# jrnerupudinho/Semi-Blind-Channel-Estimation-for-MIMO-RIS-communication-system-Using-EM-Algo

Hardware: NVIDIA B200
Metric: EM channel-estimation trials/sec (higher is better)
Workload: dtype f64

## Files before the change

semi-blind-channel-estimation-for-mimo-ris-communication-system-using-em-algo_b200/csrc/abi.cu:

```cuda
#include <atomic>
#include <mutex>
#include <vector>
#include <stdio.h>
#include <string.h>

#include "common.cuh"

namespace sbce {

static std::atomic<long long> g_launches{0};
void count_launch(int n) { g_launches.fetch_add(n, std::memory_order_relaxed); }

struct PhaseSpan { int phase; cudaEvent_t a, b; };
static std::atomic<bool> g_prof_on{false};
static std::vector<PhaseSpan> g_spans;
static std::vector<cudaEvent_t> g_event_pool;
static std::mutex g_prof_mu;

static cudaEvent_t prof_event() {
    {
        std::lock_guard<std::mutex> lock(g_prof_mu);
        if (!g_event_pool.empty()) { cudaEvent_t e = g_event_pool.back(); g_event_pool.pop_back(); return e; }
    }
    cudaEvent_t e;
    cudaEventCreate(&e);
    return e;
}

struct PhaseScope {
    bool on; int phase; cudaStream_t s; cudaEvent_t a;
    PhaseScope(int ph, cudaStream_t st) : on(g_prof_on.load(std::memory_order_relaxed)), phase(ph), s(st), a(nullptr) {
        if (on) { a = prof_event(); cudaEventRecord(a, s); }
    }
    ~PhaseScope() {
        if (on) {
            cudaEvent_t b = prof_event();
            cudaEventRecord(b, s);
            std::lock_guard<std::mutex> lock(g_prof_mu);
            g_spans.push_back({phase, a, b});
        }
    }
};

static int make_dims(const sbce_cfg* c, Dims* d, bool with_estep = true) {
    if (!c) return SBCE_E_NULL;
    if (c->N < 1 || c->n_tx < 1 || c->n_rx < 1 || c->T_p < 0 || c->T_d < 1 || c->itera < 0 || c->batch < 0)
        return SBCE_E_SHAPE;
    int sq = 0;
    if (c->M == 4) sq = 2; else if (c->M == 16) sq = 4; else if (c->M == 64) sq = 8; else return SBCE_E_UNSUPPORTED;
    if (c->n_tx > 8 || c->n_rx > 8) return SBCE_E_UNSUPPORTED;
    if (!gram_supports(c->N + 1, c->n_tx, c->n_rx)) return SBCE_E_UNSUPPORTED;
    if (c->n_tx <= 4 && !(c->n_rx <= 4 || c->n_rx == 6 || c->n_rx == 8)) return SBCE_E_UNSUPPORTED;
    if (c->mode < SBCE_MODE_SOFT || c->mode > SBCE_MODE_MMSE) return SBCE_E_UNSUPPORTED;
    if (with_estep) {
        const int bits = c->n_tx * (sq == 2 ? 2 : (sq == 4 ? 4 : 6));
        const bool tree = c->mode == SBCE_MODE_SOFT || c->mode == SBCE_MODE_HARD;
        if (tree && c->n_tx > 4 && bits > 24) return SBCE_E_UNSUPPORTED;
        if ((c->mode == SBCE_MODE_ZF || c->mode == SBCE_MODE_MMSE) && bits > 30) return SBCE_E_UNSUPPORTED;
    }
    d->N = c->N; d->N1 = c->N + 1; d->n_tx = c->n_tx; d->n_rx = c->n_rx; d->M = c->M; d->sqM = sq;
    d->bitsM = (sq == 2 ? 2 : (sq == 4 ? 4 : 6));
    d->T_p = c->T_p; d->T_d = c->T_d; d->itera = c->itera;
    d->L = d->N1 * c->n_tx;
    d->Lp = (d->L + 7) & ~7;
    d->RP = (c->n_rx + 3) & ~3;
    d->Ltot = d->Lp + d->RP;
    d->mode = c->mode; d->flags = c->flags; d->p1 = c->partition_p1;
    d->psi_shared = (c->flags & SBCE_FLAG_PSI_SHARED) ? 1 : 0;
    d->psiP_shared = (c->flags & (SBCE_FLAG_PSI_SHARED | SBCE_FLAG_PSIP_SHARED)) ? 1 : 0;
    d->rec = qr_record_doubles(c->n_tx);
    if (c->mode == SBCE_MODE_PM || c->mode == SBCE_MODE_PM_BETA) {
        if (c->partition_p1 < 1 || c->partition_p1 > c->n_tx) return SBCE_E_SHAPE;
    }
    if (c->mode >= SBCE_MODE_PM && c->n_rx < c->n_tx) return SBCE_E_UNSUPPORTED;
    if (c->flags & SBCE_FLAG_SUPERIMPOSED) {
        if (c->T_p != 0) return SBCE_E_SHAPE;
        if (c->mode != SBCE_MODE_SOFT && c->mode != SBCE_MODE_HARD) return SBCE_E_UNSUPPORTED;
    }
    return 0;
}

static inline size_t al(size_t x) { return (x + 255) & ~(size_t)255; }

size_t carve_workspace(const Dims& d, int nb, void* base, Workspace* ws) {
    size_t off = 0;
    char* p = (char*)base;
    auto take = [&](size_t bytes) { char* r = p ? p + off : nullptr; off += al(bytes); return r; };
    const size_t B = (size_t)nb;
    ws->stat_m = (double*)take(B * d.T_d * d.n_tx * 16);
    ws->stat_R = (double*)take(B * d.T_d * d.n_tx * d.n_tx * 16);
    ws->pil_m = (double*)take(B * d.T_p * d.n_tx * 16 + 16);
    ws->pil_R = (double*)take(B * d.T_p * d.n_tx * d.n_tx * 16 + 16);
    ws->qr = (double*)take(B * d.T_d * d.rec * 8);
    ws->lse_sym = (double*)take(B * d.T_d * 8);
    ws->Gp = (double*)take(B * d.Ltot * d.Lp * 16);
    ws->G = (double*)take(B * d.Ltot * d.Lp * 16);
    ws->active = (int32_t*)take(B * 4);
    ws->stat = (int32_t*)take(B * 4);
    ws->kscratch = (int32_t*)take(B * d.T_d * 4);
    ws->thbuf = (double*)take(B * d.Lp * d.n_rx * 16);
    ws->psiw = (double*)take(B * d.T_p * d.N1 * 16 + 16);
    ws->ls_scale = (double*)take(B * d.N1 * 8);
    ws->ls_rep = (int32_t*)take(B * d.N1 * 4);
    ws->bytes = off;
    return off;
}

#define CK(x)                                  \
    do {                                       \
        cudaError_t _e = (x);                  \
        if (_e != cudaSuccess) return (int)_e; \
    } while (0)

cudaError_t launch_pm_stats(const Dims& d, int nb, const double* Yd, const double* PsiD, const double* theta,
                            const double* varn, const int32_t* active, double* stat_m, double* stat_R,
                            int32_t* kstar, cudaStream_t s);

static int estep_dispatch(const Dims& d, int nb, const double* Yd, const double* PsiD, const double* theta,
                          const double* varn, const int32_t* active, Workspace& ws, double* stat_m, double* stat_R,
                          int32_t* kstar, double* lse_sym, const double* Xoff, cudaStream_t s) {
    if (d.mode == SBCE_MODE_SOFT || d.mode == SBCE_MODE_HARD) {
        {
            PhaseScope ps(SBCE_PHASE_HEFF_QR, s);
            CK(launch_heff_qr(d, nb, Yd, PsiD, theta, active, Xoff, ws.qr, s));
        }
        {
            PhaseScope ps(SBCE_PHASE_ENUM, s);
            CK(launch_enum(d, nb, ws.qr, varn, active, stat_m, stat_R, kstar, lse_sym, s));
            if (Xoff) CK(launch_superimpose_stats(d, nb, Xoff, active, stat_m, stat_R, s));
        }
    } else {
        PhaseScope ps(SBCE_PHASE_ENUM, s);
        CK(launch_pm_stats(d, nb, Yd, PsiD, theta, varn, active, stat_m, stat_R, kstar, s));
    }
    return 0;
}

static inline Dims pilot_dims(const Dims& d) { Dims dp = d; dp.psi_shared = d.psiP_shared; return dp; }

static int em_chunk(const Dims& d, int nb, const sbce_io& io, Workspace& ws, cudaStream_t s) {
    const bool tree = d.mode == SBCE_MODE_SOFT || d.mode == SBCE_MODE_HARD;
    const bool decides = tree || d.mode == SBCE_MODE_ZF || d.mode == SBCE_MODE_MMSE;
    if (io.kstar && !decides) CK(cudaMemsetAsync(io.kstar, 0xFF, (size_t)nb * d.T_d * sizeof(int32_t), s));
    {
        PhaseScope ps(SBCE_PHASE_SETUP, s);
        CK(launch_init_state(d, nb, io.theta0, io.theta, ws.active, ws.stat, io.iters, io.llf, io.lse, s));
        CK(launch_pilot_stats(d, nb, io.Xp, ws.pil_m, ws.pil_R, s));
        CK(launch_normal_equations(pilot_dims(d), nb, io.PsiP, d.T_p, io.Yp, ws.pil_m, ws.pil_R, nullptr, ws.Gp, nullptr, s));
    }
    for (int l = 0; l < d.itera; ++l) {
        int rc = estep_dispatch(d, nb, io.Yd, io.PsiD, io.theta, io.varn, ws.active, ws, ws.stat_m, ws.stat_R,
                                io.kstar, ws.lse_sym, (d.flags & SBCE_FLAG_SUPERIMPOSED) ? io.Xp : nullptr, s);
        if (rc) return rc;
        {
            PhaseScope ps(SBCE_PHASE_GRAM, s);
            CK(launch_normal_equations(d, nb, io.PsiD, d.T_d, io.Yd, ws.stat_m, ws.stat_R, ws.Gp, ws.G, ws.active,
                                       s));
        }
        {
            PhaseScope ps(SBCE_PHASE_CHOL, s);
            CK(launch_chol_solve(d, nb, ws.G, io.theta, ws.active, ws.stat, ws.thbuf, s));
        }
        {
            PhaseScope ps(SBCE_PHASE_METRICS, s);
            CK(launch_after_iteration(d, nb, l, io.theta, io.h_true, io.Yp, io.Yd, io.PsiP, io.PsiD, io.Xp,
                                      io.Xd_true, io.varn, tree ? ws.lse_sym : nullptr, ws.active, io.iters, io.llf,
                                      io.lse, s));
        }
    }
    {
        PhaseScope ps(SBCE_PHASE_METRICS, s);
        CK(launch_final_metrics(d, nb, io.theta, io.h_true, ws.stat, io.nmse, io.status, s));
    }
    return 0;
}

static sbce_io offset_io(const Dims& d, const sbce_io& io, size_t b0) {
    sbce_io o = io;
    const size_t Ln = (size_t)d.L * d.n_rx * 2;
    auto adv = [](const double* p, size_t n) { return p ? p + n : p; };
    auto advw = [](double* p, size_t n) { return p ? p + n : p; };
    o.Yd = adv(io.Yd, b0 * d.T_d * d.n_rx * 2);
    o.Yp = adv(io.Yp, b0 * d.T_p * d.n_rx * 2);
    if (!d.psi_shared) o.PsiD = adv(io.PsiD, b0 * d.T_d * d.N1 * 2);
    if (!d.psiP_shared) o.PsiP = adv(io.PsiP, b0 * d.T_p * d.N1 * 2);
    o.Xp = adv(io.Xp, b0 * ((d.flags & SBCE_FLAG_SUPERIMPOSED) ? d.T_d : d.T_p) * d.n_tx * 2);
    o.theta0 = adv(io.theta0, b0 * Ln);
    o.varn = adv(io.varn, b0);
    o.h_true = adv(io.h_true, b0 * Ln);
    o.Xd_true = adv(io.Xd_true, b0 * d.T_d * d.n_tx * 2);
    o.theta = advw(io.theta, b0 * Ln);
    o.kstar = io.kstar ? io.kstar + b0 * d.T_d : nullptr;
    o.llf = advw(io.llf, b0 * d.itera);
    o.lse = advw(io.lse, b0 * d.itera);
    o.nmse = advw(io.nmse, b0);
    o.iters = io.iters ? io.iters + b0 : nullptr;
    o.status = io.status ? io.status + b0 : nullptr;
    return o;
}

static int check_io(const Dims& d, const sbce_io* io) {
    if (!io) return SBCE_E_NULL;
    if (!io->Yd || !io->PsiD || !io->varn || !io->theta) return SBCE_E_NULL;
    if (d.T_p > 0 && (!io->Yp || !io->PsiP || !io->Xp)) return SBCE_E_NULL;
    if (!(d.flags & SBCE_FLAG_ZERO_START) && !io->theta0) return SBCE_E_NULL;
    if ((d.flags & SBCE_FLAG_GENIE_STOP) && !io->h_true) return SBCE_E_NULL;
    if ((d.flags & SBCE_FLAG_SUPERIMPOSED) && !io->Xp) return SBCE_E_NULL;
    return 0;
}

}

using namespace sbce;

extern "C" {

int sbce_version(void) { return SBCE_VERSION; }

const char* sbce_error_string(int code) {
    switch (code) {
        case 0: return "ok";
        case SBCE_E_NULL: return "required pointer is null";
        case SBCE_E_SHAPE: return "invalid shape parameter";
        case SBCE_E_UNSUPPORTED: return "unsupported configuration (n_tx,n_rx<=8; n_tx<=4: n_rx in {1,2,3,4,6,8}; M in {4,16,64}; N+1+n_tx^2<=908; exhaustive modes with n_tx>4 need n_tx*log2(M)<=24)";
        case SBCE_E_WORKSPACE: return "workspace too small for one trial";
        case SBCE_E_NODEVICE: return "no CUDA device";
        default: return code > 0 ? cudaGetErrorString((cudaError_t)code) : "unknown error";
    }
}

int sbce_device_count(void) {
    int n = 0;
    if (cudaGetDeviceCount(&n) != cudaSuccess) { cudaGetLastError(); return 0; }
    return n;
}

int sbce_workspace_bytes(const sbce_cfg* cfg, int32_t trials_in_flight, size_t* bytes) {
    Dims d;
    int rc = make_dims(cfg, &d);
    if (rc) return rc;
    if (!bytes) return SBCE_E_NULL;
    if (trials_in_flight < 1) return SBCE_E_SHAPE;
    Workspace ws;
    *bytes = carve_workspace(d, trials_in_flight, nullptr, &ws);
    return 0;
}

constexpr int SBCE_MAX_CHUNK = 65535;
static int trials_fitting(const Dims& d, size_t bytes, int want) {
    Workspace ws;
    if (want > SBCE_MAX_CHUNK) want = SBCE_MAX_CHUNK;
    if (carve_workspace(d, 1, nullptr, &ws) > bytes) return 0;
    int lo = 1, hi = want;
    while (lo < hi) {
        int mid = (lo + hi + 1) / 2;
        if (carve_workspace(d, mid, nullptr, &ws) <= bytes) lo = mid; else hi = mid - 1;
    }
    return lo;
}

int sbce_em_batch(const sbce_cfg* cfg, const sbce_io* io, void* workspace, size_t workspace_bytes, void* stream) {
    Dims d;
    int rc = make_dims(cfg, &d);
    if (rc) return rc;
    rc = check_io(d, io);
    if (rc) return rc;
    if (cfg->batch == 0) return 0;
    if (!workspace) return SBCE_E_NULL;
    const int chunk = trials_fitting(d, workspace_bytes, cfg->batch);
    if (chunk < 1) return SBCE_E_WORKSPACE;
    cudaStream_t s = (cudaStream_t)stream;
    for (int b0 = 0; b0 < cfg->batch; b0 += chunk) {
        const int nb = (cfg->batch - b0 < chunk) ? cfg->batch - b0 : chunk;
        Workspace ws;
        carve_workspace(d, nb, workspace, &ws);
        sbce_io o = offset_io(d, *io, (size_t)b0);
        rc = em_chunk(d, nb, o, ws, s);
        if (rc) return rc;
    }
    return 0;
}

int sbce_estep(const sbce_cfg* cfg, const sbce_io* io, const double* theta, double* stat_m, double* stat_R,
               int32_t* kstar, double* lse_sym, void* workspace, size_t workspace_bytes, void* stream) {
    Dims d;
    int rc = make_dims(cfg, &d);
    if (rc) return rc;
    if (!io || !io->Yd || !io->PsiD || !io->varn || !theta || !stat_m || !stat_R || !workspace) return SBCE_E_NULL;
    if (cfg->batch == 0) return 0;
    const int chunk = trials_fitting(d, workspace_bytes, cfg->batch);
    if (chunk < 1) return SBCE_E_WORKSPACE;
    cudaStream_t s = (cudaStream_t)stream;
    for (int b0 = 0; b0 < cfg->batch; b0 += chunk) {
        const int nb = (cfg->batch - b0 < chunk) ? cfg->batch - b0 : chunk;
        Workspace ws;
        carve_workspace(d, nb, workspace, &ws);
        sbce_io o = offset_io(d, *io, (size_t)b0);
        const size_t sb = (size_t)b0 * d.T_d;
        rc = estep_dispatch(d, nb, o.Yd, o.PsiD, theta + (size_t)b0 * d.L * d.n_rx * 2, o.varn, nullptr, ws,
                            stat_m + sb * d.n_tx * 2, stat_R + sb * d.n_tx * d.n_tx * 2, kstar ? kstar + sb : nullptr,
                            lse_sym ? lse_sym + sb : nullptr, (d.flags & SBCE_FLAG_SUPERIMPOSED) ? o.Xp : nullptr, s);
        if (rc) return rc;
    }
    return 0;
}

int sbce_mstep(const sbce_cfg* cfg, const sbce_io* io, const double* stat_m, const double* stat_R, double* theta_out,
               int32_t* status, void* workspace, size_t workspace_bytes, void* stream) {
    Dims d;
    int rc = make_dims(cfg, &d, false);
    if (rc) return rc;
    if (!io || !io->Yd || !io->PsiD || !stat_m || !stat_R || !theta_out || !workspace) return SBCE_E_NULL;
    if (d.T_p > 0 && (!io->Yp || !io->PsiP || !io->Xp)) return SBCE_E_NULL;
    if (cfg->batch == 0) return 0;
    const int chunk = trials_fitting(d, workspace_bytes, cfg->batch);
    if (chunk < 1) return SBCE_E_WORKSPACE;
    cudaStream_t s = (cudaStream_t)stream;
    for (int b0 = 0; b0 < cfg->batch; b0 += chunk) {
        const int nb = (cfg->batch - b0 < chunk) ? cfg->batch - b0 : chunk;
        Workspace ws;
        carve_workspace(d, nb, workspace, &ws);
        sbce_io o = offset_io(d, *io, (size_t)b0);
        const size_t sb = (size_t)b0 * d.T_d;
        CK(cudaMemsetAsync(ws.stat, 0, (size_t)nb * 4, s));
        CK(launch_pilot_stats(d, nb, o.Xp, ws.pil_m, ws.pil_R, s));
        CK(launch_normal_equations(pilot_dims(d), nb, o.PsiP, d.T_p, o.Yp, ws.pil_m, ws.pil_R, nullptr, ws.Gp, nullptr, s));
        CK(launch_normal_equations(d, nb, o.PsiD, d.T_d, o.Yd, stat_m + sb * d.n_tx * 2,
                                   stat_R + sb * d.n_tx * d.n_tx * 2, ws.Gp, ws.G, nullptr, s));
        CK(launch_chol_solve(d, nb, ws.G, theta_out + (size_t)b0 * d.L * d.n_rx * 2, nullptr, ws.stat, ws.thbuf, s));
        if (status) CK(cudaMemcpyAsync(status + b0, ws.stat, (size_t)nb * 4, cudaMemcpyDeviceToDevice, s));
    }
    return 0;
}

int sbce_accumulate_nmse(const double* nmse, const int32_t* status, int32_t batch, double* acc, void* stream) {
    if (!nmse || !acc) return SBCE_E_NULL;
    CK(launch_accumulate_nmse(nmse, status, batch, acc, (cudaStream_t)stream));
    return 0;
}

int sbce_generate_batch(const sbce_cfg* cfg, const sbce_gen* gen, const sbce_io* io, void* stream) {
    Dims d;
    int rc = make_dims(cfg, &d, false);
    if (rc) return rc;
    if (!gen || !io) return SBCE_E_NULL;
    if (!io->h_true || !io->Xd_true || !io->PsiD || !io->Yd || !io->varn) return SBCE_E_NULL;
    if (d.T_p > 0 && (!io->Xp || !io->PsiP || !io->Yp)) return SBCE_E_NULL;
    if (gen->pilot_design < SBCE_PILOTS_PM || gen->pilot_design > SBCE_PILOTS_TOP) return SBCE_E_UNSUPPORTED;
    if (gen->data_phases < SBCE_PHASES_RANDOM || gen->data_phases > SBCE_PHASES_DFT) return SBCE_E_UNSUPPORTED;
    if (cfg->batch == 0) return 0;
    for (int b0 = 0; b0 < cfg->batch; b0 += SBCE_MAX_CHUNK) {
        const int nb = (cfg->batch - b0 < SBCE_MAX_CHUNK) ? cfg->batch - b0 : SBCE_MAX_CHUNK;
        sbce_gen g = *gen;
        g.trial0 = gen->trial0 + b0;
        const sbce_io o = offset_io(d, *io, (size_t)b0);
        CK(launch_generate(d, nb, &g, o, (double*)o.h_true, (double*)o.Xp, (double*)o.Xd_true, (double*)o.PsiP,
                           (double*)o.PsiD, (double*)o.Yp, (double*)o.Yd, (cudaStream_t)stream));
    }
    return 0;
}

int sbce_ls_start(const sbce_cfg* cfg, const sbce_io* io, double* theta0, int32_t* status, void* workspace,
                  size_t workspace_bytes, void* stream) {
    Dims d;
    int rc = make_dims(cfg, &d, false);
    if (rc) return rc;
    if (!io || !io->Yp || !io->PsiP || !io->Xp || !theta0 || !workspace) return SBCE_E_NULL;
    if (d.T_p < 1) return SBCE_E_SHAPE;
    if (cfg->batch == 0) return 0;
    const int chunk = trials_fitting(d, workspace_bytes, cfg->batch);
    if (chunk < 1) return SBCE_E_WORKSPACE;
    for (int b0 = 0; b0 < cfg->batch; b0 += chunk) {
        const int nb = (cfg->batch - b0 < chunk) ? cfg->batch - b0 : chunk;
        Workspace ws;
        carve_workspace(d, nb, workspace, &ws);
        sbce_io o = offset_io(d, *io, (size_t)b0);
        CK(launch_ls_start(pilot_dims(d), nb, o, theta0 + (size_t)b0 * d.L * d.n_rx * 2, status ? status + b0 : nullptr, ws,
                           (cudaStream_t)stream));
    }
    return 0;
}

int sbce_accumulate_ser(const sbce_cfg* cfg, const int32_t* kstar, const double* Xd_true, int32_t batch, double* acc,
                        void* stream) {
    Dims d;
    int rc = make_dims(cfg, &d, false);
    if (rc) return rc;
    if (!kstar || !Xd_true || !acc) return SBCE_E_NULL;
    if (d.n_tx * d.bitsM > 30) return SBCE_E_UNSUPPORTED;
    CK(launch_accumulate_ser(d, batch, kstar, Xd_true, acc, (cudaStream_t)stream));
    return 0;
}

int sbce_measure_fp64_peak(double* tflops, double* seconds) {
    CK(run_fp64_peak(tflops, seconds));
    return 0;
}

int sbce_profile_begin(void) {
    std::lock_guard<std::mutex> lock(g_prof_mu);
    for (auto& sp : g_spans) { g_event_pool.push_back(sp.a); g_event_pool.push_back(sp.b); }
    g_spans.clear();
    g_prof_on.store(true);
    return 0;
}

int sbce_profile_end(double* ms_per_phase, int64_t* spans_per_phase, int32_t n_phases) {
    std::lock_guard<std::mutex> lock(g_prof_mu);
    g_prof_on.store(false);
    if (!ms_per_phase || n_phases < 1) return SBCE_E_NULL;
    for (int i = 0; i < n_phases; ++i) { ms_per_phase[i] = 0.0; if (spans_per_phase) spans_per_phase[i] = 0; }
    for (auto& sp : g_spans) {
        CK(cudaEventSynchronize(sp.b));
        float ms = 0.f;
        CK(cudaEventElapsedTime(&ms, sp.a, sp.b));
        if (sp.phase >= 0 && sp.phase < n_phases) {
            ms_per_phase[sp.phase] += ms;
            if (spans_per_phase) spans_per_phase[sp.phase] += 1;
        }
        g_event_pool.push_back(sp.a);
        g_event_pool.push_back(sp.b);
    }
    g_spans.clear();
    return 0;
}

int64_t sbce_launch_count(int32_t reset) {
    long long v = g_launches.load();
    if (reset) g_launches.store(0);
    return (int64_t)v;
}

namespace {
struct GraphSlot {
    unsigned long long key = 0;
    int seen = 0;
    long long launches = 0;
    cudaGraphExec_t exec = nullptr;
    unsigned long long stamp = 0;
};
struct DevPool {
    void* p = nullptr;
    size_t cap = 0;
    cudaStream_t stream = nullptr;
    cudaStream_t copy = nullptr;
    cudaEvent_t ev[2] = {nullptr, nullptr};
    GraphSlot graphs[4];
    unsigned long long clock = 0;
    std::mutex mu;
};

unsigned long long fnv1a(const void* data, size_t n, unsigned long long h) {
    const unsigned char* p = (const unsigned char*)data;
    for (size_t i = 0; i < n; ++i) { h ^= p[i]; h *= 1099511628211ull; }
    return h;
}
constexpr int SBCE_MAX_DEVICES = 64;
DevPool g_pool[SBCE_MAX_DEVICES];

int pool_get(int dev, size_t bytes, DevPool** out) {
    DevPool& P = g_pool[dev];
    if (!P.stream) {
        CK(cudaStreamCreateWithFlags(&P.stream, cudaStreamNonBlocking));
        CK(cudaStreamCreateWithFlags(&P.copy, cudaStreamNonBlocking));
        CK(cudaEventCreateWithFlags(&P.ev[0], cudaEventDisableTiming));
        CK(cudaEventCreateWithFlags(&P.ev[1], cudaEventDisableTiming));
    }
    if (P.cap < bytes) {
        for (GraphSlot& g : P.graphs) {
            if (g.exec) cudaGraphExecDestroy(g.exec);
            g = GraphSlot();
        }
        if (P.p) CK(cudaFree(P.p));
        P.p = nullptr;
        P.cap = 0;
        CK(cudaMalloc(&P.p, bytes));
        P.cap = bytes;
    }
    *out = &P;
    return 0;
}

struct DeviceGuard {
    int prev = -1;
    bool armed = false;
    int enter(int dev) {
        CK(cudaGetDevice(&prev));
        armed = true;
        if (prev != dev) CK(cudaSetDevice(dev));
        return 0;
    }
    ~DeviceGuard() {
        if (armed) { int cur = -1; if (cudaGetDevice(&cur) == cudaSuccess && cur != prev) cudaSetDevice(prev); }
    }
};

struct DrainGuard {
    DevPool* P = nullptr;
    ~DrainGuard() {
        if (P) {
            if (P->copy) cudaStreamSynchronize(P->copy);
            if (P->stream) cudaStreamSynchronize(P->stream);
        }
    }
};

constexpr int SBCE_HOST_SPLIT_MIN_BATCH = 1184;
}

int sbce_host_split_threshold(void) { return SBCE_HOST_SPLIT_MIN_BATCH; }

static int run_half(DevPool* P, const sbce_cfg* c2, const sbce_io* o, void* ws, size_t ws_bytes) {
    cudaStream_t s = P->stream;
    if (g_prof_on.load(std::memory_order_relaxed)) return sbce_em_batch(c2, o, ws, ws_bytes, (void*)s);
    unsigned long long key = fnv1a(c2, sizeof(*c2), 1469598103934665603ull);
    key = fnv1a(o, sizeof(*o), key);
    key = fnv1a(&ws, sizeof(ws), key);
    key = fnv1a(&ws_bytes, sizeof(ws_bytes), key);
    GraphSlot* slot = nullptr;
    GraphSlot* lru = &P->graphs[0];
    for (GraphSlot& g : P->graphs) {
        if (g.key == key && g.seen > 0) slot = &g;
        if (g.stamp < lru->stamp) lru = &g;
    }
    if (!slot) {
        if (lru->exec) { cudaGraphExecDestroy(lru->exec); lru->exec = nullptr; }
        lru->key = key; lru->seen = 1; lru->launches = 0; lru->stamp = ++P->clock;
        return sbce_em_batch(c2, o, ws, ws_bytes, (void*)s);
    }
    slot->stamp = ++P->clock;
    if (!slot->exec) {
        const long long before = g_launches.load();
        cudaGraph_t graph = nullptr;
        if (cudaStreamBeginCapture(s, cudaStreamCaptureModeThreadLocal) != cudaSuccess) {
            cudaGetLastError();
            return sbce_em_batch(c2, o, ws, ws_bytes, (void*)s);
        }
        const int rc = sbce_em_batch(c2, o, ws, ws_bytes, (void*)s);
        const cudaError_t ce = cudaStreamEndCapture(s, &graph);
        const long long captured = g_launches.load() - before;
        g_launches.fetch_sub(captured);
        if (rc != 0 || ce != cudaSuccess || graph == nullptr) {
            if (graph) cudaGraphDestroy(graph);
            cudaGetLastError();
            slot->seen = 0;
            slot->key = 0;
            return rc ? rc : sbce_em_batch(c2, o, ws, ws_bytes, (void*)s);
        }
        const cudaError_t ie = cudaGraphInstantiate(&slot->exec, graph, 0);
        cudaGraphDestroy(graph);
        if (ie != cudaSuccess) {
            cudaGetLastError();
            slot->exec = nullptr; slot->seen = 0; slot->key = 0;
            return sbce_em_batch(c2, o, ws, ws_bytes, (void*)s);
        }
        slot->launches = captured;
    }
    slot->seen += 1;
    CK(cudaGraphLaunch(slot->exec, s));
    count_launch((int)slot->launches);
    return 0;
}

int sbce_em_batch_host(const sbce_cfg* cfg, const sbce_io* io, int32_t device) {
    Dims d;
    int rc = make_dims(cfg, &d);
    if (rc) return rc;
    rc = check_io(d, io);
    if (rc) return rc;
    if (cfg->batch == 0) return 0;
    if (device < 0 || device >= SBCE_MAX_DEVICES || device >= sbce_device_count()) return SBCE_E_NODEVICE;
    std::lock_guard<std::mutex> lock(g_pool[device].mu);
    DeviceGuard dg;
    rc = dg.enter(device);
    if (rc) return rc;
    const size_t B = (size_t)cfg->batch;
    const size_t Ln = (size_t)d.L * d.n_rx * 16;
    const size_t psiB = d.psi_shared ? 1 : B, psiPB = d.psiP_shared ? 1 : B;
    struct Seg { const void* h; size_t bytes; size_t off; bool in; void* hout; };
    size_t off = 0;
    auto seg = [&](const void* h, size_t bytes, bool in, void* hout) {
        Seg s{h, bytes, off, in, hout};
        if (h || hout) off += al(bytes);
        return s;
    };
    Seg sYd = seg(io->Yd, B * d.T_d * d.n_rx * 16, true, nullptr);
    Seg sYp = seg(io->Yp, B * d.T_p * d.n_rx * 16, true, nullptr);
    Seg sPd = seg(io->PsiD, psiB * d.T_d * d.N1 * 16, true, nullptr);
    Seg sPp = seg(io->PsiP, psiPB * d.T_p * d.N1 * 16, true, nullptr);
    const size_t xpT = (d.flags & SBCE_FLAG_SUPERIMPOSED) ? d.T_d : d.T_p;
    Seg sXp = seg(io->Xp, B * xpT * d.n_tx * 16, true, nullptr);
    Seg sT0 = seg(io->theta0, B * Ln, true, nullptr);
    Seg sVn = seg(io->varn, B * 8, true, nullptr);
    Seg sHt = seg(io->h_true, B * Ln, true, nullptr);
    Seg sXd = seg(io->Xd_true, B * d.T_d * d.n_tx * 16, true, nullptr);
    Seg oTh = seg(nullptr, B * Ln, false, io->theta);
    Seg oKs = seg(nullptr, B * d.T_d * 4, false, io->kstar);
    Seg oLl = seg(nullptr, B * d.itera * 8, false, io->llf);
    Seg oLs = seg(nullptr, B * d.itera * 8, false, io->lse);
    Seg oNm = seg(nullptr, B * 8, false, io->nmse);
    Seg oIt = seg(nullptr, B * 4, false, io->iters);
    Seg oSt = seg(nullptr, B * 4, false, io->status);
    const size_t io_bytes = off;
    size_t freeb = 0, totalb = 0;
    CK(cudaMemGetInfo(&freeb, &totalb));
    size_t per1 = 0, perB = 0;
    { Workspace w; per1 = carve_workspace(d, 1, nullptr, &w); perB = carve_workspace(d, cfg->batch, nullptr, &w); }
    size_t budget = (freeb + g_pool[device].cap) / 3;
    if (budget < per1) budget = per1;
    size_t ws_bytes = perB < budget ? perB : budget;
    DevPool* P = nullptr;
    rc = pool_get(device, io_bytes + ws_bytes + 256, &P);
    if (rc) return rc;
    DrainGuard drain;
    drain.P = P;
    char* base = (char*)P->p;
    cudaStream_t s = P->stream;
    sbce_io dio;
    memset(&dio, 0, sizeof(dio));
    auto dp = [&](const Seg& q) { return (q.h || q.hout) ? (double*)(base + q.off) : nullptr; };
    dio.Yd = dp(sYd); dio.Yp = dp(sYp); dio.PsiD = dp(sPd); dio.PsiP = dp(sPp); dio.Xp = dp(sXp);
    dio.theta0 = dp(sT0); dio.varn = dp(sVn); dio.h_true = dp(sHt); dio.Xd_true = dp(sXd);
    dio.theta = dp(oTh); dio.kstar = (int32_t*)dp(oKs); dio.llf = dp(oLl); dio.lse = dp(oLs); dio.nmse = dp(oNm);
    dio.iters = (int32_t*)dp(oIt); dio.status = (int32_t*)dp(oSt);

    const int nhalf = (cfg->batch >= SBCE_HOST_SPLIT_MIN_BATCH) ? 2 : 1;
    const int half = (cfg->batch + nhalf - 1) / nhalf;
    struct Part { Seg* q; size_t per_trial; };
    Part ins[] = {{&sYd, (size_t)d.T_d * d.n_rx * 16}, {&sYp, (size_t)d.T_p * d.n_rx * 16},
                  {&sPd, d.psi_shared ? 0 : (size_t)d.T_d * d.N1 * 16}, {&sPp, d.psiP_shared ? 0 : (size_t)d.T_p * d.N1 * 16},
                  {&sXp, xpT * d.n_tx * 16}, {&sT0, Ln}, {&sVn, 8}, {&sHt, Ln},
                  {&sXd, (size_t)d.T_d * d.n_tx * 16}};
    Part outs[] = {{&oTh, Ln}, {&oKs, (size_t)d.T_d * 4}, {&oLl, (size_t)d.itera * 8}, {&oLs, (size_t)d.itera * 8},
                   {&oNm, 8}, {&oIt, 4}, {&oSt, 4}};
    for (int hf = 0; hf < nhalf; ++hf) {
        const size_t b0 = (size_t)hf * half;
        const size_t nb = (b0 + half <= B) ? (size_t)half : B - b0;
        for (Part& pt : ins) {
            if (!pt.q->h || !pt.q->bytes) continue;
            if (pt.per_trial == 0) {
                if (hf == 0) CK(cudaMemcpyAsync(base + pt.q->off, pt.q->h, pt.q->bytes, cudaMemcpyHostToDevice, P->copy));
            } else {
                CK(cudaMemcpyAsync(base + pt.q->off + b0 * pt.per_trial, (const char*)pt.q->h + b0 * pt.per_trial,
                                   nb * pt.per_trial, cudaMemcpyHostToDevice, P->copy));
            }
        }
        CK(cudaEventRecord(P->ev[hf], P->copy));
    }
    for (int hf = 0; hf < nhalf; ++hf) {
        const size_t b0 = (size_t)hf * half;
        const size_t nb = (b0 + half <= B) ? (size_t)half : B - b0;
        CK(cudaStreamWaitEvent(s, P->ev[hf], 0));
        sbce_cfg c2 = *cfg;
        c2.batch = (int32_t)nb;
        sbce_io o = offset_io(d, dio, b0);
        rc = run_half(P, &c2, &o, base + al(io_bytes), ws_bytes);
        if (rc) return rc;
        for (Part& pt : outs)
            if (pt.q->hout && pt.q->bytes)
                CK(cudaMemcpyAsync((char*)pt.q->hout + b0 * pt.per_trial, base + pt.q->off + b0 * pt.per_trial,
                                   nb * pt.per_trial, cudaMemcpyDeviceToHost, s));
    }
    CK(cudaStreamSynchronize(s));
    CK(cudaStreamSynchronize(P->copy));
    return 0;
}

}
```

semi-blind-channel-estimation-for-mimo-ris-communication-system-using-em-algo_b200/csrc/common.cuh:

```cuda
#pragma once

#include <cuda_runtime.h>
#include <stdint.h>

#include <atomic>

#include "../../include/sbce.h"

namespace sbce {

typedef double2 cplx;

__host__ __device__ __forceinline__ cplx mk(double re, double im) { return make_double2(re, im); }
__device__ __forceinline__ cplx cadd(cplx a, cplx b) { return mk(a.x + b.x, a.y + b.y); }
__device__ __forceinline__ cplx csub(cplx a, cplx b) { return mk(a.x - b.x, a.y - b.y); }
__device__ __forceinline__ cplx cmul(cplx a, cplx b) {
    return mk(fma(a.x, b.x, -a.y * b.y), fma(a.x, b.y, a.y * b.x));
}
__device__ __forceinline__ cplx cmulc(cplx a, cplx b) {
    return mk(fma(a.x, b.x, a.y * b.y), fma(a.y, b.x, -a.x * b.y));
}
__device__ __forceinline__ cplx cconj(cplx a) { return mk(a.x, -a.y); }
__device__ __forceinline__ cplx cscale(cplx a, double s) { return mk(a.x * s, a.y * s); }
__device__ __forceinline__ double cnorm2(cplx a) { return fma(a.x, a.x, a.y * a.y); }
__device__ __forceinline__ void cfma(cplx& acc, cplx a, cplx b) {
    acc.x = fma(a.x, b.x, acc.x);
    acc.x = fma(-a.y, b.y, acc.x);
    acc.y = fma(a.x, b.y, acc.y);
    acc.y = fma(a.y, b.x, acc.y);
}
__device__ __forceinline__ void cfmac(cplx& acc, cplx a, cplx b) {
    acc.x = fma(a.x, b.x, acc.x);
    acc.x = fma(a.y, b.y, acc.x);
    acc.y = fma(a.y, b.x, acc.y);
    acc.y = fma(-a.x, b.y, acc.y);
}
__device__ __forceinline__ void cfmsc(cplx& acc, cplx a, cplx b) {
    acc.x = fma(-a.x, b.x, acc.x);
    acc.x = fma(-a.y, b.y, acc.x);
    acc.y = fma(-a.y, b.x, acc.y);
    acc.y = fma(a.x, b.y, acc.y);
}

__device__ __forceinline__ double shfl_xor_d(double v, int m) { return __shfl_xor_sync(0xffffffffu, v, m); }
__device__ __forceinline__ double shfl_d(double v, int src) { return __shfl_sync(0xffffffffu, v, src); }
__device__ __forceinline__ double warp_sum(double v) {
#pragma unroll
    for (int o = 16; o > 0; o >>= 1) v += shfl_xor_d(v, o);
    return v;
}

constexpr int RH_MAXR = 8;

struct Dims {
    int N, N1, n_tx, n_rx, M, sqM, bitsM, T_p, T_d, itera;
    int L;
    int Lp;
    int RP;
    int Ltot;
    int mode;
    unsigned flags;
    int p1;
    int psi_shared;
    int psiP_shared;
    int rec;
};

__host__ __device__ __forceinline__ int qr_record_doubles(int n_tx) { return n_tx * (n_tx + 1) + 2 * n_tx + 2; }

struct Workspace {
    double* stat_m;
    double* stat_R;
    double* pil_m;
    double* pil_R;
    double* qr;
    double* lse_sym;
    double* Gp;
    double* G;
    int32_t* active;
    int32_t* stat;
    int32_t* kscratch;
    double* psiw;
    double* ls_scale;
    int32_t* ls_rep;
    double* thbuf;
    size_t bytes;
};

size_t carve_workspace(const Dims& d, int nb, void* base, Workspace* ws);

cudaError_t launch_pilot_stats(const Dims& d, int nb, const double* Xp, double* pil_m, double* pil_R, cudaStream_t s);
cudaError_t launch_heff_qr(const Dims& d, int nb, const double* Yd, const double* PsiD, const double* theta,
                           const int32_t* active, const double* Xoff, double* qr, cudaStream_t s);
cudaError_t launch_superimpose_stats(const Dims& d, int nb, const double* Xoff, const int32_t* active, double* stat_m,
                                     double* stat_R, cudaStream_t s);
cudaError_t launch_enum(const Dims& d, int nb, const double* qr, const double* varn, const int32_t* active,
                        double* stat_m, double* stat_R, int32_t* kstar, double* lse_sym, cudaStream_t s);
cudaError_t launch_normal_equations(const Dims& d, int nb, const double* Psi, int T, const double* Y,
                                    const double* sm, const double* sR, const double* Ginit, double* Gout,
                                    const int32_t* active, cudaStream_t s);
bool gram_supports(int N1, int n_tx, int n_rx);
cudaError_t launch_chol_solve(const Dims& d, int nb, double* G, double* theta, const int32_t* active, int32_t* stat,
                              double* th_scratch, cudaStream_t s);
cudaError_t launch_init_state(const Dims& d, int nb, const double* theta0, double* theta, int32_t* active,
                              int32_t* stat, int32_t* iters, double* llf, double* lse, cudaStream_t s);
cudaError_t launch_after_iteration(const Dims& d, int nb, int l, const double* theta, const double* h_true,
                                   const double* Yp, const double* Yd, const double* PsiP, const double* PsiD,
                                   const double* Xp, const double* Xd_true, const double* varn, const double* lse_sym,
                                   int32_t* active, int32_t* iters, double* llf, double* lse, cudaStream_t s);
cudaError_t launch_final_metrics(const Dims& d, int nb, const double* theta, const double* h_true, const int32_t* stat,
                                 double* nmse, int32_t* status, cudaStream_t s);
cudaError_t launch_accumulate_nmse(const double* nmse, const int32_t* status, int batch, double* acc, cudaStream_t s);
cudaError_t run_fp64_peak(double* tflops, double* seconds);
cudaError_t launch_generate(const Dims& d, int nb, const sbce_gen* g, const sbce_io& io, double* h_out, double* Xp_out,
                            double* Xd_out, double* PsiP_out, double* PsiD_out, double* Yp_out, double* Yd_out,
                            cudaStream_t s);
cudaError_t launch_ls_start(const Dims& d, int nb, const sbce_io& io, double* theta0, int32_t* status, Workspace& ws,
                            cudaStream_t s);
cudaError_t launch_accumulate_ser(const Dims& d, int nb, const int32_t* kstar, const double* Xd, double* acc,
                                  cudaStream_t s);

void count_launch(int n = 1);


struct SmemOptIn {
    std::atomic<size_t> have[64];
};
inline cudaError_t opt_in_smem(SmemOptIn& st, const void* kernel, size_t smem) {
    if (smem <= 48 * 1024) return cudaSuccess;
    int dev = 0;
    cudaError_t e = cudaGetDevice(&dev);
    if (e != cudaSuccess) return e;
    if (dev >= 0 && dev < 64 && st.have[dev].load(std::memory_order_relaxed) >= smem) return cudaSuccess;
    e = cudaFuncSetAttribute(kernel, cudaFuncAttributeMaxDynamicSharedMemorySize, (int)smem);
    if (e == cudaSuccess && dev >= 0 && dev < 64) st.have[dev].store(smem, std::memory_order_relaxed);
    return e;
}

}
```

semi-blind-channel-estimation-for-mimo-ris-communication-system-using-em-algo_b200/csrc/estep.cu:

```cuda
#include <math.h>

#include "common.cuh"
#include "tensor.cuh"

namespace sbce {

static __device__ __forceinline__ constexpr int cmax(int a, int b) { return a > b ? a : b; }

__global__ void k_pilot_stats(int n_tx, int total, const cplx* __restrict__ Xp, cplx* __restrict__ pm,
                              cplx* __restrict__ pR) {
    int s = blockIdx.x * blockDim.x + threadIdx.x;
    if (s >= total) return;
    const cplx* x = Xp + (size_t)s * n_tx;
    for (int i = 0; i < n_tx; ++i) {
        cplx xi = x[i];
        pm[(size_t)s * n_tx + i] = cconj(xi);
        for (int j = 0; j < n_tx; ++j) pR[((size_t)s * n_tx + i) * n_tx + j] = cmulc(x[j], xi);
    }
}

cudaError_t launch_pilot_stats(const Dims& d, int nb, const double* Xp, double* pil_m, double* pil_R, cudaStream_t s) {
    int total = nb * d.T_p;
    if (total == 0) return cudaSuccess;
    k_pilot_stats<<<(total + 127) / 128, 128, 0, s>>>(d.n_tx, total, (const cplx*)Xp, (cplx*)pil_m, (cplx*)pil_R);
    count_launch();
    return cudaGetLastError();
}

template <int NTX, int NRX>
__device__ __forceinline__ void heff_qr_finish(const Dims& d, int b, int t, cplx (&A)[cmax(NTX, NRX)][NTX],
                                               const cplx* __restrict__ Yd, const cplx* __restrict__ Xoff,
                                               double* __restrict__ qr) {
    constexpr int NR = cmax(NTX, NRX);
    cplx y[NR];
#pragma unroll
    for (int r = 0; r < NR; ++r) y[r] = (r < NRX) ? Yd[((size_t)b * d.T_d + t) * NRX + r] : mk(0.0, 0.0);
    if (Xoff != nullptr) {
        const cplx* o = Xoff + ((size_t)b * d.T_d + t) * NTX;
#pragma unroll
        for (int j = 0; j < NTX; ++j) {
            const cplx oj = o[j], noj = mk(-oj.x, -oj.y);
#pragma unroll
            for (int r = 0; r < NRX; ++r) cfma(y[r], A[r][j], noj);
        }
    }

#pragma unroll
    for (int k = 0; k < NTX; ++k) {
        double nrm2 = 0.0;
#pragma unroll
        for (int i = k; i < NR; ++i) nrm2 += cnorm2(A[i][k]);
        if (nrm2 > 0.0) {
            const double nrm = sqrt(nrm2);
            const cplx a0 = A[k][k];
            const double abs0 = sqrt(cnorm2(a0));
            const cplx phase = abs0 > 0.0 ? mk(a0.x / abs0, a0.y / abs0) : mk(1.0, 0.0);
            const cplx vk = cscale(phase, abs0 + nrm);
            const double beta = 1.0 / (nrm * (nrm + abs0));
#pragma unroll
            for (int c = k + 1; c <= NTX; ++c) {
                cplx w = mk(0.0, 0.0);
                if (c < NTX) {
                    cfmac(w, A[k][c], vk);
#pragma unroll
                    for (int i = k + 1; i < NR; ++i) cfmac(w, A[i][c], A[i][k]);
                    w = cscale(w, beta);
                    cplx nw = mk(-w.x, -w.y);
                    cfma(A[k][c], nw, vk);
#pragma unroll
                    for (int i = k + 1; i < NR; ++i) cfma(A[i][c], nw, A[i][k]);
                } else {
                    cfmac(w, y[k], vk);
#pragma unroll
                    for (int i = k + 1; i < NR; ++i) cfmac(w, y[i], A[i][k]);
                    w = cscale(w, beta);
                    cplx nw = mk(-w.x, -w.y);
                    cfma(y[k], nw, vk);
#pragma unroll
                    for (int i = k + 1; i < NR; ++i) cfma(y[i], nw, A[i][k]);
                }
            }
            const cplx rot = mk(-phase.x, phase.y);
#pragma unroll
            for (int c = k + 1; c < NTX; ++c) A[k][c] = cmul(A[k][c], rot);
            y[k] = cmul(y[k], rot);
            A[k][k] = mk(nrm, 0.0);
        } else {
            A[k][k] = mk(0.0, 0.0);
        }
    }

    double* rec = qr + ((size_t)b * d.T_d + t) * d.rec;
    int o = 0;
#pragma unroll
    for (int i = 0; i < NTX; ++i)
#pragma unroll
        for (int j = i; j < NTX; ++j) {
            rec[o++] = A[i][j].x;
            rec[o++] = (j == i) ? 0.0 : A[i][j].y;
        }
#pragma unroll
    for (int i = 0; i < NTX; ++i) {
        rec[o++] = y[i].x;
        rec[o++] = y[i].y;
    }
    double c0 = 0.0;
#pragma unroll
    for (int i = NTX; i < NR; ++i) c0 += cnorm2(y[i]);
    rec[o++] = c0;
    rec[o++] = 0.0;
}

template <int NTX, int NRX>
__global__ void __launch_bounds__(128) k_heff_qr(Dims d, const cplx* __restrict__ Yd, const cplx* __restrict__ PsiD,
                                                 const cplx* __restrict__ theta, const int32_t* __restrict__ active,
                                                 const cplx* __restrict__ Xoff, double* __restrict__ qr, int use_smem) {
    constexpr int NR = cmax(NTX, NRX);
    extern __shared__ double2 heff_smem[];
    const int b = blockIdx.y;
    if (active != nullptr && active[b] == 0) return;
    const cplx* th = theta + (size_t)b * d.L * NRX;
    if (use_smem) {
        for (int e = threadIdx.x; e < d.L * NRX; e += blockDim.x) heff_smem[e] = th[e];
        __syncthreads();
        th = heff_smem;
    }
    const int t = blockIdx.x * blockDim.x + threadIdx.x;
    if (t >= d.T_d) return;

    const cplx* psi = PsiD + ((size_t)(d.psi_shared ? 0 : b) * d.T_d + t) * d.N1;

    cplx A[NR][NTX];
#pragma unroll
    for (int r = 0; r < NR; ++r)
#pragma unroll
        for (int j = 0; j < NTX; ++j) A[r][j] = mk(0.0, 0.0);

#pragma unroll 4
    for (int n = 0; n < d.N1; ++n) {
        const cplx p = psi[n];
        const cplx* row = th + (size_t)n * NTX * NRX;
#pragma unroll
        for (int j = 0; j < NTX; ++j)
#pragma unroll
            for (int r = 0; r < NRX; ++r) cfma(A[r][j], p, row[j * NRX + r]);
    }
    heff_qr_finish<NTX, NRX>(d, b, t, A, Yd, Xoff, qr);
}

template <int NTX, int NRX>
__global__ void __launch_bounds__(128, 4) k_heff_qr_mma(Dims d, const cplx* __restrict__ Yd,
                                                        const cplx* __restrict__ PsiD, const cplx* __restrict__ theta,
                                                        const int32_t* __restrict__ active,
                                                        const cplx* __restrict__ Xoff, double* __restrict__ qr) {
    constexpr int NR = cmax(NTX, NRX);
    constexpr int NC = NTX * NRX;
    constexpr int NT = (NC + 7) / 8;
    constexpr int TS = NT * 8 + 2;
    constexpr int HS = NC + 1;
    extern __shared__ double2 heff_smem[];
    const int b = blockIdx.y;
    if (active != nullptr && active[b] == 0) return;
    const int N1 = d.N1, KP = (N1 + 7) & ~7;
    cplx* sTh = heff_smem;
    cplx* sH = sTh + KP * TS;
    {
        const cplx* th = theta + (size_t)b * d.L * NRX;
        for (int e = threadIdx.x; e < KP * TS; e += blockDim.x) {
            const int n = e / TS, c = e % TS;
            sTh[e] = (n < N1 && c < NC) ? th[n * NC + c] : mk(0.0, 0.0);
        }
    }
    __syncthreads();
    const int warp = threadIdx.x >> 5, lane = threadIdx.x & 31, g = lane >> 2, tig = lane & 3;
    const int t0 = blockIdx.x * 128 + warp * 32;
    if (t0 >= d.T_d) return;
    const cplx* psi_b = PsiD + (size_t)(d.psi_shared ? 0 : b) * d.T_d * N1;
    const cplx* prow[2][2];
#pragma unroll
    for (int mt = 0; mt < 2; ++mt)
#pragma unroll
        for (int h = 0; h < 2; ++h) prow[mt][h] = psi_b + (size_t)min(t0 + mt * 16 + g + 8 * h, d.T_d - 1) * N1;
    {
        const char* rowp = (const char*)(psi_b + (size_t)min(t0 + lane, d.T_d - 1) * N1);
        for (int o = 0; o < N1 * (int)sizeof(cplx); o += 128) asm volatile("prefetch.global.L2 [%0];" ::"l"(rowp + o));
    }
    double cr[2][NT][4], ci[2][NT][4];
#pragma unroll
    for (int mt = 0; mt < 2; ++mt)
#pragma unroll
        for (int nt = 0; nt < NT; ++nt)
#pragma unroll
            for (int e = 0; e < 4; ++e) { cr[mt][nt][e] = 0.0; ci[mt][nt][e] = 0.0; }
#pragma unroll 2
    for (int k0 = 0; k0 < KP; k0 += 8) {
        const int ka = k0 + tig, kb = ka + 4;
        const bool va = ka < N1, vb = kb < N1;
        double ar[2][4], ai[2][4];
#pragma unroll
        for (int mt = 0; mt < 2; ++mt) {
            const cplx a0 = va ? prow[mt][0][ka] : mk(0.0, 0.0), a1 = va ? prow[mt][1][ka] : mk(0.0, 0.0);
            const cplx a2 = vb ? prow[mt][0][kb] : mk(0.0, 0.0), a3 = vb ? prow[mt][1][kb] : mk(0.0, 0.0);
            ar[mt][0] = a0.x; ar[mt][1] = a1.x; ar[mt][2] = a2.x; ar[mt][3] = a3.x;
            ai[mt][0] = a0.y; ai[mt][1] = a1.y; ai[mt][2] = a2.y; ai[mt][3] = a3.y;
        }
#pragma unroll
        for (int nt = 0; nt < NT; ++nt) {
            const cplx b0 = sTh[ka * TS + 8 * nt + g], b1 = sTh[kb * TS + 8 * nt + g];
#pragma unroll
            for (int mt = 0; mt < 2; ++mt) {
                dmma16x8x8(cr[mt][nt], ar[mt], b0.x, b1.x);
                dmma16x8x8(ci[mt][nt], ar[mt], b0.y, b1.y);
                dmma16x8x8(cr[mt][nt], ai[mt], -b0.y, -b1.y);
                dmma16x8x8(ci[mt][nt], ai[mt], b0.x, b1.x);
            }
        }
    }
    cplx* H = sH + (size_t)warp * 32 * HS;
#pragma unroll
    for (int mt = 0; mt < 2; ++mt)
#pragma unroll
        for (int nt = 0; nt < NT; ++nt)
#pragma unroll
            for (int h = 0; h < 2; ++h) {
                const int row = mt * 16 + g + 8 * h, c = 8 * nt + 2 * tig;
                if (c < NC) H[row * HS + c] = mk(cr[mt][nt][2 * h], ci[mt][nt][2 * h]);
                if (c + 1 < NC) H[row * HS + c + 1] = mk(cr[mt][nt][2 * h + 1], ci[mt][nt][2 * h + 1]);
            }
    __syncwarp();
    const int t = t0 + lane;
    if (t >= d.T_d) return;
    cplx A[NR][NTX];
#pragma unroll
    for (int r = 0; r < NR; ++r)
#pragma unroll
        for (int j = 0; j < NTX; ++j) A[r][j] = (r < NRX) ? H[lane * HS + j * NRX + r] : mk(0.0, 0.0);
    heff_qr_finish<NTX, NRX>(d, b, t, A, Yd, Xoff, qr);
}

__device__ __forceinline__ double group8_sum(double v) {
    v += shfl_xor_d(v, 4);
    v += shfl_xor_d(v, 2);
    v += shfl_xor_d(v, 1);
    return v;
}

template <int NTX>
__global__ void __launch_bounds__(128) k_heff_qr_rows(Dims d, const cplx* __restrict__ Yd,
                                                      const cplx* __restrict__ PsiD, const cplx* __restrict__ theta,
                                                      const int32_t* __restrict__ active,
                                                      const cplx* __restrict__ Xoff, double* __restrict__ qr) {
    const int b = blockIdx.y;
    if (active != nullptr && active[b] == 0) return;
    const int r = threadIdx.x & 7;
    const int tq = blockIdx.x * (blockDim.x >> 3) + (threadIdx.x >> 3);
    const bool tv = tq < d.T_d;
    const int t = tv ? tq : d.T_d - 1;
    const int nrx = d.n_rx;
    const bool rv = r < nrx;
    const int rr = rv ? r : 0;

    const cplx* psi = PsiD + ((size_t)(d.psi_shared ? 0 : b) * d.T_d + t) * d.N1;
    const cplx* th = theta + (size_t)b * d.L * nrx;

    cplx A[NTX + 1];
#pragma unroll
    for (int j = 0; j <= NTX; ++j) A[j] = mk(0.0, 0.0);
#pragma unroll 2
    for (int n = 0; n < d.N1; ++n) {
        const cplx p = psi[n];
        const cplx* row = th + (size_t)n * NTX * nrx + rr;
#pragma unroll
        for (int j = 0; j < NTX; ++j) cfma(A[j], p, __ldg(&row[j * nrx]));
    }
    A[NTX] = Yd[((size_t)b * d.T_d + t) * nrx + rr];
    if (Xoff != nullptr) {
        const cplx* o = Xoff + ((size_t)b * d.T_d + t) * NTX;
#pragma unroll
        for (int j = 0; j < NTX; ++j) {
            const cplx oj = o[j];
            cfma(A[NTX], A[j], mk(-oj.x, -oj.y));
        }
    }
    if (!rv) {
#pragma unroll
        for (int j = 0; j <= NTX; ++j) A[j] = mk(0.0, 0.0);
    }

#pragma unroll
    for (int k = 0; k < NTX; ++k) {
        const double nrm2 = group8_sum(r >= k ? cnorm2(A[k]) : 0.0);
        const bool ok = nrm2 > 0.0;
        const double nrm = sqrt(nrm2);
        const int src = (threadIdx.x & 24) + k;
        const cplx a0 = mk(shfl_d(A[k].x, src), shfl_d(A[k].y, src));
        const double abs0 = sqrt(cnorm2(a0));
        const cplx phase = abs0 > 0.0 ? mk(a0.x / abs0, a0.y / abs0) : mk(1.0, 0.0);
        const cplx vk = cscale(phase, abs0 + nrm);
        const double beta = ok ? 1.0 / (nrm * (nrm + abs0)) : 0.0;
        const cplx vr = (r == k) ? vk : (r > k ? A[k] : mk(0.0, 0.0));
#pragma unroll
        for (int c = k + 1; c <= NTX; ++c) {
            cplx w = mk(0.0, 0.0);
            cfmac(w, A[c], vr);
            w = mk(group8_sum(w.x) * beta, group8_sum(w.y) * beta);
            const cplx nw = mk(-w.x, -w.y);
            cfma(A[c], nw, vr);
        }
        if (r == k) {
            const cplx rot = mk(-phase.x, phase.y);
#pragma unroll
            for (int c = k + 1; c <= NTX; ++c) A[c] = cmul(A[c], rot);
            A[k] = mk(ok ? nrm : 0.0, 0.0);
        }
    }
    const double c0 = group8_sum(r >= NTX ? cnorm2(A[NTX]) : 0.0);
    if (!tv) return;
    double* rec = qr + ((size_t)b * d.T_d + t) * d.rec;
    if (r < NTX) {
        double* o = rec + 2 * (r * NTX - (r * (r - 1)) / 2);
#pragma unroll
        for (int j = 0; j < NTX; ++j)
            if (j >= r) {
                o[2 * (j - r)] = A[j].x;
                o[2 * (j - r) + 1] = (j == r) ? 0.0 : A[j].y;
            }
        rec[NTX * (NTX + 1) + 2 * r] = A[NTX].x;
        rec[NTX * (NTX + 1) + 2 * r + 1] = A[NTX].y;
    }
    if (r == 0) {
        rec[NTX * (NTX + 1) + 2 * NTX] = c0;
        rec[NTX * (NTX + 1) + 2 * NTX + 1] = 0.0;
    }
}

constexpr double SBCE_THR = 64.0;
constexpr int ENUM_QCAP = 1024;

template <int NTX, int SQM>
struct EnumT {
    static constexpr int M = SQM * SQM;
    static constexpr int BITS = (SQM == 2 ? 2 : (SQM == 4 ? 4 : 6));
    static constexpr int HB = BITS / 2;
    static constexpr int NODE_STREAMS = NTX - 1;
    static constexpr int PLWANT = (5 + BITS - 1) / BITS;
    static constexpr int PL = NODE_STREAMS < PLWANT ? NODE_STREAMS : PLWANT;
    static constexpr int NPREF = 1 << (BITS * PL);
    static constexpr int NPAIR = NTX * (NTX - 1) / 2;
    static constexpr int NPAIR1 = NPAIR > 0 ? NPAIR : 1;
    static constexpr int NACC = 1 + 3 * NTX + 2 * NPAIR;
    static constexpr int O_TAB = 0;
    static constexpr int O_G = O_TAB + 2 * NPAIR1 * M;
    static constexpr int O_YT = O_G + NTX * SQM;
    static constexpr int O_C0 = O_YT + 2 * NTX;
    static constexpr int O_ACC = O_C0 + 1;
    static constexpr int O_AREF = O_ACC + NACC;
    static constexpr int O_S2 = O_AREF + 1;
    static constexpr int O_CNT = O_S2 + 1;
    static constexpr int O_Q = O_CNT + 1;
    static constexpr int O_SCR = O_Q + ENUM_QCAP / 2;
    static constexpr int WS_DOUBLES = ((O_SCR + NACC * 32) + 1) & ~1;

    __device__ __forceinline__ static double pam(int a) { return (double)(2 * a - SQM + 1); }
    __device__ __forceinline__ static cplx cval(int m) { return mk(pam(m & (SQM - 1)), pam(m >> HB)); }
    __device__ __forceinline__ static int pair(int i, int s) { return s * (s - 1) / 2 + i; }

    __device__ __forceinline__ static int slice(double v, const double* gs, double& dist) {
        int a = 0;
        double e = v - gs[0];
        dist = e * e;
#pragma unroll
        for (int q = 1; q < SQM; ++q) {
            e = v - gs[q];
            const double dq = e * e;
            if (dq < dist) { dist = dq; a = q; }
        }
        return a;
    }

    __device__ __forceinline__ static double fold(double v, double r) {
        double a = fabs(v);
        if (SQM == 8) a = fabs(a - 4.0 * r);
        if (SQM >= 4) a = fabs(a - 2.0 * r);
        return a - r;
    }
};

template <int NTX, int SQM>
__device__ __noinline__ void enum_flush(double* ws, double warp_best) {
    typedef EnumT<NTX, SQM> E;
    constexpr int M = E::M;
    const int lane = threadIdx.x & 31;
    __syncwarp();
    int* cntp = (int*)(ws + E::O_CNT);
    const int n = min(*cntp, ENUM_QCAP);
    const int* q = (const int*)(ws + E::O_Q);
    const cplx* tab = (const cplx*)(ws + E::O_TAB);
    const double* g = ws + E::O_G;
    const double inv_s2 = ws[E::O_S2];
    double aref = ws[E::O_AREF];
    if (warp_best < aref) {
        const double f = exp((warp_best - aref) * inv_s2);
        for (int i = lane; i < E::NACC; i += 32) ws[E::O_ACC + i] *= f;
        aref = warp_best;
    }
    double* A = ws + E::O_ACC;
    if (n <= 2) {
        constexpr int LG = (SQM == 2 ? 1 : (SQM == 4 ? 2 : 3));
        const int a = lane & (SQM - 1);
        const bool isQ = (lane >> LG) & 1;
        const double pq = E::pam(a);
        for (int e = 0; e < n; ++e) {
            const int code = q[e];
            double base = ws[E::O_C0];
            cplx t0;
            {
                cplx acc[NTX];
#pragma unroll
                for (int i = 0; i < NTX; ++i) acc[i] = mk(ws[E::O_YT + 2 * i], ws[E::O_YT + 2 * i + 1]);
#pragma unroll
                for (int s = NTX - 1; s >= 1; --s) {
                    const int m = (code >> (E::BITS * (NTX - 1 - s))) & (M - 1);
                    const double eI = acc[s].x - g[s * SQM + (m & (SQM - 1))];
                    const double eQ = acc[s].y - g[s * SQM + (m >> E::HB)];
                    base += fma(eI, eI, eQ * eQ);
#pragma unroll
                    for (int i = 0; i < NTX; ++i)
                        if (i < s) acc[i] = csub(acc[i], tab[E::pair(i, s) * M + m]);
                }
                t0 = acc[0];
            }
            const double ev = (isQ ? t0.y : t0.x) - g[a];
            const double dd = ev * ev;
            double mn = dd;
#pragma unroll
            for (int o = SQM / 2; o > 0; o >>= 1) mn = fmin(mn, shfl_xor_d(mn, o));
            const double w = exp((mn - dd) * inv_s2);
            double s0 = w, s1 = pq * w, s2 = pq * pq * w;
#pragma unroll
            for (int o = SQM / 2; o > 0; o >>= 1) {
                s0 += shfl_xor_d(s0, o);
                s1 += shfl_xor_d(s1, o);
                s2 += shfl_xor_d(s2, o);
            }
            const double o0 = shfl_xor_d(s0, SQM), o1 = shfl_xor_d(s1, SQM), o2 = shfl_xor_d(s2, SQM);
            const double om = shfl_xor_d(mn, SQM);
            const double EI = isQ ? o0 : s0, A1 = isQ ? o1 : s1, A2 = isQ ? o2 : s2, minI = isQ ? om : mn;
            const double EQ = isQ ? s0 : o0, B1 = isQ ? s1 : o1, B2 = isQ ? s2 : o2, minQ = isQ ? mn : om;
            const double W = exp((aref - (base + minI + minQ)) * inv_s2);
            const double E0 = W * EI * EQ;
            const cplx F0 = mk(W * A1 * EQ, -W * EI * B1);
            const double Q0 = W * (A2 * EQ + EI * B2);
            constexpr int NR = (E::NACC + 31) / 32;
            double mine[NR];
#pragma unroll
            for (int r = 0; r < NR; ++r) mine[r] = 0.0;
            auto add = [&](int idx, double v) { if ((idx & 31) == lane) mine[idx >> 5] = v; };
            add(0, E0);
            add(1, F0.x);
            add(1 + NTX, F0.y);
            add(1 + 2 * NTX, Q0);
#pragma unroll
            for (int s = 1; s < NTX; ++s) {
                const cplx xs = E::cval((code >> (E::BITS * (NTX - 1 - s))) & (M - 1));
                add(1 + s, E0 * xs.x);
                add(1 + NTX + s, -E0 * xs.y);
                add(1 + 2 * NTX + s, E0 * cnorm2(xs));
                const cplx v = cmul(F0, xs);
                add(1 + 3 * NTX + 2 * E::pair(0, s), v.x);
                add(1 + 3 * NTX + 2 * E::pair(0, s) + 1, v.y);
#pragma unroll
                for (int i = 1; i < NTX; ++i)
                    if (i < s) {
                        const cplx xi = E::cval((code >> (E::BITS * (NTX - 1 - i))) & (M - 1));
                        const cplx cx = cmulc(xs, xi);
                        add(1 + 3 * NTX + 2 * E::pair(i, s), E0 * cx.x);
                        add(1 + 3 * NTX + 2 * E::pair(i, s) + 1, E0 * cx.y);
                    }
            }
#pragma unroll
            for (int r = 0; r < NR; ++r)
                if (32 * r + lane < E::NACC) A[32 * r + lane] += mine[r];
            __syncwarp();
        }
        if (lane == 0) {
            ws[E::O_AREF] = aref;
            *cntp = 0;
        }
        __syncwarp();
        return;
    }
    double* scr = ws + E::O_SCR;
    int nround = 0;
    auto radd = [&](int idx, double v) { scr[idx * 32 + lane] = v; };
    for (int e0 = 0; e0 < n; e0 += 32) {
        const int e = e0 + lane;
        const bool have = e < n;
        nround = min(32, n - e0);
        const int code = have ? q[e] : 0;
        cplx t0;
        double base = ws[E::O_C0];
        {
            cplx acc[NTX];
#pragma unroll
            for (int i = 0; i < NTX; ++i) acc[i] = mk(ws[E::O_YT + 2 * i], ws[E::O_YT + 2 * i + 1]);
#pragma unroll
            for (int s = NTX - 1; s >= 1; --s) {
                const int m = (code >> (E::BITS * (NTX - 1 - s))) & (M - 1);
                const double eI = acc[s].x - g[s * SQM + (m & (SQM - 1))];
                const double eQ = acc[s].y - g[s * SQM + (m >> E::HB)];
                base += fma(eI, eI, eQ * eQ);
#pragma unroll
                for (int i = 0; i < NTX; ++i)
                    if (i < s) acc[i] = csub(acc[i], tab[E::pair(i, s) * M + m]);
            }
            t0 = acc[0];
        }
        double minI = 1e300, minQ = 1e300;
#pragma unroll
        for (int a = 0; a < SQM; ++a) {
            const double eI = t0.x - g[a], eQ = t0.y - g[a];
            minI = fmin(minI, eI * eI);
            minQ = fmin(minQ, eQ * eQ);
        }
        const double W = have ? exp((aref - (base + minI + minQ)) * inv_s2) : 0.0;
        double EI = 0, A1 = 0, A2 = 0, EQ = 0, B1 = 0, B2 = 0;
#pragma unroll 1
        for (int a = 0; a < SQM; ++a) {
            const double pq = E::pam(a);
            const double eI = t0.x - g[a], eQ = t0.y - g[a];
            const double wI = exp((minI - eI * eI) * inv_s2), wQ = exp((minQ - eQ * eQ) * inv_s2);
            EI += wI; A1 = fma(pq, wI, A1); A2 = fma(pq * pq, wI, A2);
            EQ += wQ; B1 = fma(pq, wQ, B1); B2 = fma(pq * pq, wQ, B2);
        }
        const double E0 = W * EI * EQ;
        const cplx F0 = mk(W * A1 * EQ, -W * EI * B1);
        const double Q0 = W * (A2 * EQ + EI * B2);
        radd(0, E0);
        radd(1, F0.x);
        radd(1 + NTX, F0.y);
        radd(1 + 2 * NTX, Q0);
#pragma unroll
        for (int s = 1; s < NTX; ++s) {
            const cplx xs = E::cval((code >> (E::BITS * (NTX - 1 - s))) & (M - 1));
            radd(1 + s, E0 * xs.x);
            radd(1 + NTX + s, -E0 * xs.y);
            radd(1 + 2 * NTX + s, E0 * cnorm2(xs));
            const cplx v = cmul(F0, xs);
            radd(1 + 3 * NTX + 2 * E::pair(0, s), v.x);
            radd(1 + 3 * NTX + 2 * E::pair(0, s) + 1, v.y);
#pragma unroll
            for (int i = 1; i < NTX; ++i)
                if (i < s) {
                    const cplx xi = E::cval((code >> (E::BITS * (NTX - 1 - i))) & (M - 1));
                    const cplx cx = cmulc(xs, xi);
                    radd(1 + 3 * NTX + 2 * E::pair(i, s), E0 * cx.x);
                    radd(1 + 3 * NTX + 2 * E::pair(i, s) + 1, E0 * cx.y);
                }
        }
        __syncwarp();
        for (int i = lane; i < E::NACC; i += 32) {
            double acc = 0.0;
            for (int e2 = 0; e2 < nround; ++e2) acc += scr[i * 32 + e2];
            A[i] += acc;
        }
        __syncwarp();
    }
    __syncwarp();
    if (lane == 0) {
        ws[E::O_AREF] = aref;
        *cntp = 0;
    }
    __syncwarp();
}

template <int NTX, int SQM, bool HARD>
struct Scan {
    typedef EnumT<NTX, SQM> E;
    static constexpr int M = E::M;
    double* ws;
    const cplx* tab;
    const double* g;
    double r0;
    double thr;
    double best, lim;
    int bestk;
    bool prune;

    __device__ __forceinline__ void leaf(cplx t0, double nb, int code) {
        const double fI = E::fold(t0.x, r0), fQ = E::fold(t0.y, r0);
        const double nodemin = fma(fI, fI, fma(fQ, fQ, nb));
        if (nodemin <= lim) {
            if (nodemin <= best) {
                double dI, dQ;
                const int iI = E::slice(t0.x, g, dI), iQ = E::slice(t0.y, g, dQ);
                const double val = nb + dI + dQ;
                const int k = code + ((iQ * SQM + iI) << (E::BITS * (NTX - 1)));
                if (val < best || (val == best && k < bestk)) {
                    best = val;
                    bestk = k;
                    lim = HARD ? val : val + thr;
                }
            }
            if (!HARD) {
                int* cntp = (int*)(ws + E::O_CNT);
                const int slot = atomicAdd(cntp, 1);
                if (slot < ENUM_QCAP) ((int*)(ws + E::O_Q))[slot] = code;
            }
        }
    }

    __device__ __forceinline__ void maybe_flush() {
        if (!HARD) {
            __syncwarp();
            const int c = *(volatile int*)(ws + E::O_CNT);
            if (c > ENUM_QCAP - 32 * SQM) {
                double wb = best;
#pragma unroll
                for (int o = 16; o > 0; o >>= 1) wb = fmin(wb, shfl_xor_d(wb, o));
                enum_flush<NTX, SQM>(ws, wb);
            }
        }
    }


    template <int S_>
    __device__ __forceinline__ void inner(const cplx (&acc)[NTX], double base, int code, cplx r01, bool dead) {
        dead = dead || (prune && base > lim);
        if constexpr (S_ == 0) {
            if (!dead) leaf(acc[0], base, code);
        } else if constexpr (S_ == 1) {
            if (__all_sync(0xffffffffu, dead)) return;
            const double* g1 = g + SQM;
            double dI1[SQM];
#pragma unroll
            for (int a = 0; a < SQM; ++a) {
                const double eI = acc[1].x - g1[a];
                dI1[a] = eI * eI;
            }
#pragma unroll 1
            for (int iQ = 0; iQ < SQM; ++iQ) {
                const double eQ = acc[1].y - g1[iQ];
                const double bq = base + __dmul_rn(eQ, eQ);
                const bool deadq = dead || (prune && bq > lim);
                if (__all_sync(0xffffffffu, deadq)) continue;
                const double pQ = E::pam(iQ);
                const cplx tq = mk(fma(pQ, r01.y, acc[0].x), fma(-pQ, r01.x, acc[0].y));
                const int cq = code + ((iQ * SQM) << (E::BITS * (NTX - 2)));
                if (!deadq) {
#pragma unroll
                    for (int iI = 0; iI < SQM; ++iI) {
                        const double pI = E::pam(iI);
                        const cplx t0 = mk(fma(-pI, r01.x, tq.x), fma(-pI, r01.y, tq.y));
                        leaf(t0, bq + dI1[iI], cq + (iI << (E::BITS * (NTX - 2))));
                    }
                }
                maybe_flush();
            }
        } else {
            if (__all_sync(0xffffffffu, dead)) return;
#pragma unroll 1
            for (int m = 0; m < M; ++m) {
                const double* gs = g + S_ * SQM;
                const double eI = acc[S_].x - gs[m & (SQM - 1)];
                const double eQ = acc[S_].y - gs[m >> E::HB];
                const double nb = base + fma(eI, eI, eQ * eQ);
                cplx nacc[NTX];
#pragma unroll
                for (int i = 0; i < NTX; ++i) nacc[i] = (i < S_) ? csub(acc[i], tab[E::pair(i, S_) * M + m]) : acc[i];
                inner<S_ - 1>(nacc, nb, code + (m << (E::BITS * (NTX - 1 - S_))), r01, dead);
            }
        }
    }

    template <int S_, int LEFT>
    __device__ __forceinline__ void prefix(const cplx (&acc)[NTX], double base, int code, int p, cplx r01, bool dead) {
        if constexpr (LEFT == 0) {
            inner<S_>(acc, base, code, r01, dead);
        } else {
            const int m = (p >> (E::BITS * (LEFT - 1))) & (M - 1);
            const double* gs = g + S_ * SQM;
            const double eI = acc[S_].x - gs[m & (SQM - 1)];
            const double eQ = acc[S_].y - gs[m >> E::HB];
            const double nb = base + fma(eI, eI, eQ * eQ);
            cplx nacc[NTX];
#pragma unroll
            for (int i = 0; i < NTX; ++i) nacc[i] = (i < S_) ? csub(acc[i], tab[E::pair(i, S_) * M + m]) : acc[i];
            prefix<S_ - 1, LEFT - 1>(nacc, nb, code + (m << (E::BITS * (NTX - 1 - S_))), p, r01, dead);
        }
    }
};

template <int NTX, int SQM, bool HARD, int WARPS>
__global__ void __launch_bounds__(WARPS * 32, (NTX > 4 ? 2 : 4)) k_enum(Dims d, const double* __restrict__ qr,
                                                     const double* __restrict__ varn,
                                                     const int32_t* __restrict__ active, cplx* __restrict__ stat_m,
                                                     cplx* __restrict__ stat_R, int32_t* __restrict__ kstar,
                                                     double* __restrict__ lse_sym) {
    typedef EnumT<NTX, SQM> E;
    constexpr int M = E::M;
    extern __shared__ __align__(16) double enum_smem[];
    const int b = blockIdx.y;
    const int warp = threadIdx.x >> 5, lane = threadIdx.x & 31;
    const int t = blockIdx.x * WARPS + warp;
    if (t >= d.T_d) return;
    const double* grec = qr + ((size_t)b * d.T_d + t) * d.rec;
    const int32_t act = (active != nullptr) ? active[b] : 1;
    const double vn = varn[b];
    const double rec0 = (lane < d.rec) ? grec[lane] : 0.0;
    if (act == 0) return;

    double* ws = enum_smem + (size_t)warp * E::WS_DOUBLES;
    cplx* tab = (cplx*)(ws + E::O_TAB);
    double* g = ws + E::O_G;
    const double* rec = ws + E::O_SCR;
    {
        if (lane < d.rec) ws[E::O_SCR + lane] = rec0;
        for (int i = lane + 32; i < d.rec; i += 32) ws[E::O_SCR + i] = grec[i];
        __syncwarp();
    }
    cplx yt[NTX];
    cplx r01 = mk(0.0, 0.0);
    double r00;
    {
        cplx Rm[NTX][NTX];
        int o = 0;
#pragma unroll
        for (int i = 0; i < NTX; ++i)
#pragma unroll
            for (int j = i; j < NTX; ++j) {
                Rm[i][j] = mk(rec[o], rec[o + 1]);
                o += 2;
            }
#pragma unroll
        for (int i = 0; i < NTX; ++i) {
            yt[i] = mk(rec[o], rec[o + 1]);
            o += 2;
        }
        r00 = Rm[0][0].x;
        if (NTX > 1) r01 = Rm[0][NTX > 1 ? 1 : 0];
#pragma unroll
        for (int s = 1; s < NTX; ++s)
#pragma unroll
            for (int i = 0; i < s; ++i)
                for (int m = lane; m < M; m += 32) tab[E::pair(i, s) * M + m] = cmul(Rm[i][s], E::cval(m));
        if (lane < NTX * SQM) {
            const int s = lane / SQM, a = lane % SQM;
            double dd = 0.0;
#pragma unroll
            for (int q = 0; q < NTX; ++q)
                if (q == s) dd = Rm[q][q].x;
            g[lane] = dd * E::pam(a);
        }
    }
    const double c0 = rec[NTX * (NTX + 1) + 2 * NTX];
    const double s2 = vn * vn, inv_s2 = 1.0 / s2;
    if (lane == 0) {
#pragma unroll
        for (int i = 0; i < NTX; ++i) {
            ws[E::O_YT + 2 * i] = yt[i].x;
            ws[E::O_YT + 2 * i + 1] = yt[i].y;
        }
        ws[E::O_C0] = c0;
        ws[E::O_AREF] = 1e300;
        ws[E::O_S2] = inv_s2;
        *(int*)(ws + E::O_CNT) = 0;
    }
    for (int i = lane; i < E::NACC; i += 32) ws[E::O_ACC + i] = 0.0;
    __syncwarp();

    Scan<NTX, SQM, HARD> sc;
    sc.ws = ws;
    sc.tab = tab;
    sc.g = g;
    sc.r0 = r00;
    sc.thr = SBCE_THR * s2;
    sc.prune = (d.flags & SBCE_FLAG_FULL_SCAN) == 0;
    {
        cplx acc[NTX];
#pragma unroll
        for (int i = 0; i < NTX; ++i) acc[i] = yt[i];
        double base = c0;
        int k = 0;
#pragma unroll
        for (int s = NTX - 1; s >= 0; --s) {
            double dI, dQ;
            const int iI = E::slice(acc[s].x, g + s * SQM, dI), iQ = E::slice(acc[s].y, g + s * SQM, dQ);
            const int m = iQ * SQM + iI;
            base += dI + dQ;
            k += m << (E::BITS * (NTX - 1 - s));
#pragma unroll
            for (int i = 0; i < NTX; ++i)
                if (i < s) acc[i] = csub(acc[i], tab[E::pair(i, s) * M + m]);
        }
        sc.best = base;
        sc.bestk = k;
        sc.lim = HARD ? base : base + sc.thr;
    }

    unsigned top_alive = 0xffffffffu;
    constexpr int TOP_SHIFT = E::BITS * (E::PL - 1);
    if (E::PL >= 2 && sc.prune) {
        bool a = false;
        if (lane < M) {
            const double* gs = g + (NTX - 1) * SQM;
            const double eI = yt[NTX - 1].x - gs[lane & (SQM - 1)];
            const double eQ = yt[NTX - 1].y - gs[lane >> E::HB];
            a = !(c0 + fma(eI, eI, eQ * eQ) > sc.lim);
        }
        top_alive = __ballot_sync(0xffffffffu, a);
    }
    for (int pb = 0; pb < E::NPREF; pb += 32) {
        if (E::PL >= 2) {
            const int lo = pb >> TOP_SHIFT, hi = min(pb + 31, E::NPREF - 1) >> TOP_SHIFT;
            const unsigned bits = (hi >= 31 ? 0xffffffffu : ((2u << hi) - 1u)) & ~((1u << lo) - 1u);
            if ((top_alive & bits) == 0u) continue;
        }
        const int p = pb + lane;
        const bool valid = p < E::NPREF;
        sc.template prefix<NTX - 1, E::PL>(yt, c0, 0, valid ? p : 0, r01, !valid);
    }

    double best = sc.best;
    int bestk = sc.bestk;
#pragma unroll
    for (int o = 16; o > 0; o >>= 1) {
        const double ob = shfl_xor_d(best, o);
        const int ok = __shfl_xor_sync(0xffffffffu, bestk, o);
        if (ob < best || (ob == best && ok < bestk)) { best = ob; bestk = ok; }
    }
    const size_t sidx = (size_t)b * d.T_d + t;
    if (kstar != nullptr && lane == 0) kstar[sidx] = bestk;

    bool collapsed = HARD;
    double S = 0.0;
    if (!HARD) {
        enum_flush<NTX, SQM>(ws, best);
        S = ws[E::O_ACC];
        if (!(S > 0.0) || !isfinite(S)) collapsed = true;
    }
    if (collapsed) {
        if (lane == 0) {
            cplx xs[NTX];
#pragma unroll
            for (int s = 0; s < NTX; ++s) xs[s] = E::cval((bestk >> (E::BITS * (NTX - 1 - s))) & (M - 1));
#pragma unroll
            for (int i = 0; i < NTX; ++i) {
                stat_m[sidx * NTX + i] = cconj(xs[i]);
#pragma unroll
                for (int j = 0; j < NTX; ++j) stat_R[(sidx * NTX + i) * NTX + j] = cmulc(xs[j], xs[i]);
            }
            if (lse_sym != nullptr) lse_sym[sidx] = -best * inv_s2;
        }
        return;
    }
    {
        const double invS = 1.0 / S;
        const double* A = ws + E::O_ACC;
        for (int l = lane; l < NTX * NTX; l += 32) {
            const int i = l / NTX, j = l % NTX;
            cplx v;
            if (i == j) {
                v = mk(A[1 + 2 * NTX + j] * invS, 0.0);
            } else {
                const int lo = min(i, j), hi = max(i, j);
                const int pr = 1 + 3 * NTX + 2 * E::pair(lo, hi);
                const double a = A[pr] * invS, c = A[pr + 1] * invS;
                v = mk(a, i < j ? c : -c);
            }
            stat_R[sidx * NTX * NTX + l] = v;
        }
        if (lane < NTX) stat_m[sidx * NTX + lane] = mk(A[1 + lane] * invS, A[1 + NTX + lane] * invS);
        if (lse_sym != nullptr && lane == 0) lse_sym[sidx] = -ws[E::O_AREF] * inv_s2 + log(S);
    }
}

__global__ void k_superimpose_stats(Dims d, int nb, const cplx* __restrict__ Xoff, const int32_t* __restrict__ active,
                                    cplx* __restrict__ stat_m, cplx* __restrict__ stat_R) {
    const int s = blockIdx.x * blockDim.x + threadIdx.x;
    if (s >= nb * d.T_d) return;
    if (active != nullptr && active[s / d.T_d] == 0) return;
    const int n = d.n_tx;
    const cplx* o = Xoff + (size_t)s * n;
    cplx* m = stat_m + (size_t)s * n;
    cplx* R = stat_R + (size_t)s * n * n;
    for (int i = 0; i < n; ++i)
        for (int j = 0; j < n; ++j) {
            cplx v = R[i * n + j];
            cfma(v, m[i], o[j]);
            v = cadd(v, cconj(cmul(o[i], m[j])));
            v = cadd(v, cmulc(o[j], o[i]));
            R[i * n + j] = v;
        }
    for (int i = 0; i < n; ++i) m[i] = cadd(m[i], cconj(o[i]));
}

cudaError_t launch_superimpose_stats(const Dims& d, int nb, const double* Xoff, const int32_t* active, double* stat_m,
                                     double* stat_R, cudaStream_t s) {
    const int total = nb * d.T_d;
    k_superimpose_stats<<<(total + 127) / 128, 128, 0, s>>>(d, nb, (const cplx*)Xoff, active, (cplx*)stat_m, (cplx*)stat_R);
    count_launch();
    return cudaGetLastError();
}

template <int NTX, int NRX>
static cudaError_t run_heff(const Dims& d, int nb, const double* Yd, const double* PsiD, const double* theta,
                            const int32_t* active, const double* Xoff, double* qr, cudaStream_t s) {
    static SmemOptIn optin_mma, optin;
    dim3 grid((d.T_d + 127) / 128, nb);
    constexpr int NC = NTX * NRX, NT = (NC + 7) / 8;
    const int KP = (d.N1 + 7) & ~7;
    const size_t smem_mma = sizeof(cplx) * ((size_t)KP * (NT * 8 + 2) + 4 * 32 * (NC + 1));
    if (NC >= 8 && d.N1 >= 16 && smem_mma <= 100 * 1024) {
        cudaError_t e = opt_in_smem(optin_mma, (const void*)k_heff_qr_mma<NTX, NRX>, smem_mma);
        if (e != cudaSuccess) return e;
        k_heff_qr_mma<NTX, NRX><<<grid, 128, smem_mma, s>>>(d, (const cplx*)Yd, (const cplx*)PsiD, (const cplx*)theta,
                                                            active, (const cplx*)Xoff, qr);
        count_launch();
        return cudaGetLastError();
    }
    size_t smem = sizeof(cplx) * (size_t)d.L * NRX;
    const int use_smem = smem <= 64 * 1024;
    if (!use_smem) smem = 0;
    cudaError_t e = opt_in_smem(optin, (const void*)k_heff_qr<NTX, NRX>, smem);
    if (e != cudaSuccess) return e;
    k_heff_qr<NTX, NRX><<<grid, 128, smem, s>>>(d, (const cplx*)Yd, (const cplx*)PsiD, (const cplx*)theta, active,
                                                (const cplx*)Xoff, qr, use_smem);
    count_launch();
    return cudaGetLastError();
}

template <int NTX>
static cudaError_t run_heff_ntx(const Dims& d, int nb, const double* Yd, const double* PsiD, const double* theta,
                                const int32_t* active, const double* Xoff, double* qr, cudaStream_t s) {
    switch (d.n_rx) {
        case 1: return run_heff<NTX, 1>(d, nb, Yd, PsiD, theta, active, Xoff, qr, s);
        case 2: return run_heff<NTX, 2>(d, nb, Yd, PsiD, theta, active, Xoff, qr, s);
        case 3: return run_heff<NTX, 3>(d, nb, Yd, PsiD, theta, active, Xoff, qr, s);
        case 4: return run_heff<NTX, 4>(d, nb, Yd, PsiD, theta, active, Xoff, qr, s);
        case 6: return run_heff<NTX, 6>(d, nb, Yd, PsiD, theta, active, Xoff, qr, s);
        case 8: return run_heff<NTX, 8>(d, nb, Yd, PsiD, theta, active, Xoff, qr, s);
        default: return cudaErrorInvalidValue;
    }
}

template <int NTX, int SQM>
static cudaError_t run_enum(const Dims& d, int nb, const double* qr, const double* varn, const int32_t* active,
                            double* stat_m, double* stat_R, int32_t* kstar, double* lse_sym, cudaStream_t s) {
    constexpr int WARPS = 4;
    dim3 grid((d.T_d + WARPS - 1) / WARPS, nb);
    constexpr size_t smem = sizeof(double) * WARPS * EnumT<NTX, SQM>::WS_DOUBLES;
    static SmemOptIn optin_hard, optin_soft;
    cudaError_t e;
    if (d.mode == SBCE_MODE_HARD) {
        e = opt_in_smem(optin_hard, (const void*)k_enum<NTX, SQM, true, WARPS>, smem);
        if (e != cudaSuccess) return e;
        k_enum<NTX, SQM, true, WARPS><<<grid, WARPS * 32, smem, s>>>(d, qr, varn, active, (cplx*)stat_m,
                                                                      (cplx*)stat_R, kstar, lse_sym);
    } else {
        e = opt_in_smem(optin_soft, (const void*)k_enum<NTX, SQM, false, WARPS>, smem);
        if (e != cudaSuccess) return e;
        k_enum<NTX, SQM, false, WARPS><<<grid, WARPS * 32, smem, s>>>(d, qr, varn, active, (cplx*)stat_m,
                                                                       (cplx*)stat_R, kstar, lse_sym);
    }
    count_launch();
    return cudaGetLastError();
}

template <int NTX>
static cudaError_t run_heff_rows(const Dims& d, int nb, const double* Yd, const double* PsiD, const double* theta,
                                 const int32_t* active, const double* Xoff, double* qr, cudaStream_t s) {
    dim3 grid((d.T_d + 15) / 16, nb);
    k_heff_qr_rows<NTX><<<grid, 128, 0, s>>>(d, (const cplx*)Yd, (const cplx*)PsiD, (const cplx*)theta, active,
                                             (const cplx*)Xoff, qr);
    count_launch();
    return cudaGetLastError();
}

template <int NTX>
static cudaError_t run_enum_wide(const Dims& d, int nb, const double* qr, const double* varn, const int32_t* active,
                                 double* stat_m, double* stat_R, int32_t* kstar, double* lse_sym, cudaStream_t s) {
    if (d.sqM == 2) return run_enum<NTX, 2>(d, nb, qr, varn, active, stat_m, stat_R, kstar, lse_sym, s);
    if constexpr (NTX <= 6) {
        if (d.sqM == 4) return run_enum<NTX, 4>(d, nb, qr, varn, active, stat_m, stat_R, kstar, lse_sym, s);
    }
    return cudaErrorInvalidValue;
}

template <int NTX>
static cudaError_t run_enum_ntx(const Dims& d, int nb, const double* qr, const double* varn, const int32_t* active,
                                double* stat_m, double* stat_R, int32_t* kstar, double* lse_sym, cudaStream_t s) {
    switch (d.sqM) {
        case 2: return run_enum<NTX, 2>(d, nb, qr, varn, active, stat_m, stat_R, kstar, lse_sym, s);
        case 4: return run_enum<NTX, 4>(d, nb, qr, varn, active, stat_m, stat_R, kstar, lse_sym, s);
        case 8: return run_enum<NTX, 8>(d, nb, qr, varn, active, stat_m, stat_R, kstar, lse_sym, s);
        default: return cudaErrorInvalidValue;
    }
}

cudaError_t launch_heff_qr(const Dims& d, int nb, const double* Yd, const double* PsiD, const double* theta,
                           const int32_t* active, const double* Xoff, double* qr, cudaStream_t s) {
    switch (d.n_tx) {
        case 1: return run_heff_ntx<1>(d, nb, Yd, PsiD, theta, active, Xoff, qr, s);
        case 2: return run_heff_ntx<2>(d, nb, Yd, PsiD, theta, active, Xoff, qr, s);
        case 3: return run_heff_ntx<3>(d, nb, Yd, PsiD, theta, active, Xoff, qr, s);
        case 4: return run_heff_ntx<4>(d, nb, Yd, PsiD, theta, active, Xoff, qr, s);
        case 5: return run_heff_rows<5>(d, nb, Yd, PsiD, theta, active, Xoff, qr, s);
        case 6: return run_heff_rows<6>(d, nb, Yd, PsiD, theta, active, Xoff, qr, s);
        case 7: return run_heff_rows<7>(d, nb, Yd, PsiD, theta, active, Xoff, qr, s);
        case 8: return run_heff_rows<8>(d, nb, Yd, PsiD, theta, active, Xoff, qr, s);
        default: return cudaErrorInvalidValue;
    }
}

cudaError_t launch_enum(const Dims& d, int nb, const double* qr, const double* varn, const int32_t* active,
                        double* stat_m, double* stat_R, int32_t* kstar, double* lse_sym, cudaStream_t s) {
    switch (d.n_tx) {
        case 1: return run_enum_ntx<1>(d, nb, qr, varn, active, stat_m, stat_R, kstar, lse_sym, s);
        case 2: return run_enum_ntx<2>(d, nb, qr, varn, active, stat_m, stat_R, kstar, lse_sym, s);
        case 3: return run_enum_ntx<3>(d, nb, qr, varn, active, stat_m, stat_R, kstar, lse_sym, s);
        case 4: return run_enum_ntx<4>(d, nb, qr, varn, active, stat_m, stat_R, kstar, lse_sym, s);
        case 5: return run_enum_wide<5>(d, nb, qr, varn, active, stat_m, stat_R, kstar, lse_sym, s);
        case 6: return run_enum_wide<6>(d, nb, qr, varn, active, stat_m, stat_R, kstar, lse_sym, s);
        case 7: return run_enum_wide<7>(d, nb, qr, varn, active, stat_m, stat_R, kstar, lse_sym, s);
        case 8: return run_enum_wide<8>(d, nb, qr, varn, active, stat_m, stat_R, kstar, lse_sym, s);
        default: return cudaErrorInvalidValue;
    }
}

}
```

Measured before the change: 23350.

## Add per-lane fast enumeration path with deferred-symbol compaction for 4x16QAM

For the NTX=4, 16-QAM soft case, a new thread-per-symbol kernel handles most symbols directly. Symbols it cannot resolve are appended to a global list through warp-ballot atomics. A persistent, occupancy-sized launch of the existing warp enumeration kernel then processes only that deferred list. The aim is to avoid paying full warp-per-symbol tree enumeration for easy symbols, at the cost of an extra launch, a memset, and atomic compaction. Several multiplies are switched to __dmul_rn to keep rounding consistent between the two paths.

```diff
diff --git a/semi-blind-channel-estimation-for-mimo-ris-communication-system-using-em-algo_b200/csrc/abi.cu b/semi-blind-channel-estimation-for-mimo-ris-communication-system-using-em-algo_b200/csrc/abi.cu
--- a/semi-blind-channel-estimation-for-mimo-ris-communication-system-using-em-algo_b200/csrc/abi.cu
+++ b/semi-blind-channel-estimation-for-mimo-ris-communication-system-using-em-algo_b200/csrc/abi.cu
@@ -98,6 +98,7 @@
     ws->active = (int32_t*)take(B * 4);
     ws->stat = (int32_t*)take(B * 4);
     ws->kscratch = (int32_t*)take(B * d.T_d * 4);
+    ws->kcount = (int32_t*)take(4);
     ws->thbuf = (double*)take(B * d.Lp * d.n_rx * 16);
     ws->psiw = (double*)take(B * d.T_p * d.N1 * 16 + 16);
     ws->ls_scale = (double*)take(B * d.N1 * 8);
@@ -126,7 +127,7 @@
         }
         {
             PhaseScope ps(SBCE_PHASE_ENUM, s);
-            CK(launch_enum(d, nb, ws.qr, varn, active, stat_m, stat_R, kstar, lse_sym, s));
+            CK(launch_enum(d, nb, ws.qr, varn, active, stat_m, stat_R, kstar, lse_sym, ws.kscratch, ws.kcount, s));
             if (Xoff) CK(launch_superimpose_stats(d, nb, Xoff, active, stat_m, stat_R, s));
         }
     } else {
diff --git a/semi-blind-channel-estimation-for-mimo-ris-communication-system-using-em-algo_b200/csrc/common.cuh b/semi-blind-channel-estimation-for-mimo-ris-communication-system-using-em-algo_b200/csrc/common.cuh
--- a/semi-blind-channel-estimation-for-mimo-ris-communication-system-using-em-algo_b200/csrc/common.cuh
+++ b/semi-blind-channel-estimation-for-mimo-ris-communication-system-using-em-algo_b200/csrc/common.cuh
@@ -66,7 +66,7 @@
     int rec;
 };
 
-__host__ __device__ __forceinline__ int qr_record_doubles(int n_tx) { return n_tx * (n_tx + 1) + 2 * n_tx + 2; }
+__host__ __device__ __forceinline__ constexpr int qr_record_doubles(int n_tx) { return n_tx * (n_tx + 1) + 2 * n_tx + 2; }
 
 struct Workspace {
     double* stat_m;
@@ -80,6 +80,7 @@
     int32_t* active;
     int32_t* stat;
     int32_t* kscratch;
+    int32_t* kcount;
     double* psiw;
     double* ls_scale;
     int32_t* ls_rep;
@@ -95,7 +96,8 @@
 cudaError_t launch_superimpose_stats(const Dims& d, int nb, const double* Xoff, const int32_t* active, double* stat_m,
                                      double* stat_R, cudaStream_t s);
 cudaError_t launch_enum(const Dims& d, int nb, const double* qr, const double* varn, const int32_t* active,
-                        double* stat_m, double* stat_R, int32_t* kstar, double* lse_sym, cudaStream_t s);
+                        double* stat_m, double* stat_R, int32_t* kstar, double* lse_sym, int32_t* dlist,
+                        int32_t* dcount, cudaStream_t s);
 cudaError_t launch_normal_equations(const Dims& d, int nb, const double* Psi, int T, const double* Y,
                                     const double* sm, const double* sR, const double* Ginit, double* Gout,
                                     const int32_t* active, cudaStream_t s);
diff --git a/semi-blind-channel-estimation-for-mimo-ris-communication-system-using-em-algo_b200/csrc/estep.cu b/semi-blind-channel-estimation-for-mimo-ris-communication-system-using-em-algo_b200/csrc/estep.cu
--- a/semi-blind-channel-estimation-for-mimo-ris-communication-system-using-em-algo_b200/csrc/estep.cu
+++ b/semi-blind-channel-estimation-for-mimo-ris-communication-system-using-em-algo_b200/csrc/estep.cu
@@ -1,4 +1,7 @@
 #include <math.h>
+
+#include <algorithm>
+#include <atomic>
 
 #include "common.cuh"
 #include "tensor.cuh"
@@ -368,14 +371,156 @@
     __device__ __forceinline__ static int slice(double v, const double* gs, double& dist) {
         int a = 0;
         double e = v - gs[0];
-        dist = e * e;
+        dist = __dmul_rn(e, e);
 #pragma unroll
         for (int q = 1; q < SQM; ++q) {
             e = v - gs[q];
-            const double dq = e * e;
+            const double dq = __dmul_rn(e, e);
             if (dq < dist) { dist = dq; a = q; }
         }
         return a;
+    }
+
+
+    __device__ __forceinline__ static double step(double base, cplx a, double gI, double gQ) {
+        const double eI = a.x - gI, eQ = a.y - gQ;
+        return base + fma(eI, eI, __dmul_rn(eQ, eQ));
+    }
+    __device__ __forceinline__ static double sq(double v, double gl) {
+        const double e = v - gl;
+        return __dmul_rn(e, e);
+    }
+    __device__ __forceinline__ static cplx sep_row(cplx acc0, cplx r01, double pQ) {
+        return mk(fma(pQ, r01.y, acc0.x), fma(-pQ, r01.x, acc0.y));
+    }
+    __device__ __forceinline__ static cplx sep_leaf(cplx tq, cplx r01, double pI) {
+        return mk(fma(-pI, r01.x, tq.x), fma(-pI, r01.y, tq.y));
+    }
+    __device__ __forceinline__ static double nodemin(cplx t0, double nb, double r0) {
+        const double fI = fold(t0.x, r0), fQ = fold(t0.y, r0);
+        return fma(fI, fI, fma(fQ, fQ, nb));
+    }
+    __device__ __forceinline__ static double best_leaf(cplx t0, double nb, const double* g0, int code, int& k) {
+        double dI, dQ;
+        const int iI = slice(t0.x, g0, dI), iQ = slice(t0.y, g0, dQ);
+        k = code + ((iQ * SQM + iI) << (BITS * (NTX - 1)));
+        return nb + dI + dQ;
+    }
+    template <class Tab, class Lev>
+    __device__ __forceinline__ static double babai(const cplx (&yt)[NTX], double c0, Tab tab, Lev lev, int& k) {
+        cplx acc[NTX];
+#pragma unroll
+        for (int i = 0; i < NTX; ++i) acc[i] = yt[i];
+        double base = c0;
+        k = 0;
+#pragma unroll
+        for (int s = NTX - 1; s >= 0; --s) {
+            double gs[SQM];
+#pragma unroll
+            for (int a = 0; a < SQM; ++a) gs[a] = lev(s, a);
+            double dI, dQ;
+            const int iI = slice(acc[s].x, gs, dI), iQ = slice(acc[s].y, gs, dQ);
+            const int m = iQ * SQM + iI;
+            base += dI + dQ;
+            k += m << (BITS * (NTX - 1 - s));
+#pragma unroll
+            for (int i = 0; i < NTX; ++i)
+                if (i < s) acc[i] = csub(acc[i], tab(i, s, m));
+        }
+        return base;
+    }
+    template <class Tab, class Lev>
+    __device__ __forceinline__ static cplx node_residual(const cplx (&yt)[NTX], double c0, Tab tab, Lev lev, int code,
+                                                         double& base) {
+        cplx acc[NTX];
+#pragma unroll
+        for (int i = 0; i < NTX; ++i) acc[i] = yt[i];
+        base = c0;
+#pragma unroll
+        for (int s = NTX - 1; s >= 1; --s) {
+            const int m = (code >> (BITS * (NTX - 1 - s))) & (M - 1);
+            base = step(base, acc[s], lev(s, m & (SQM - 1)), lev(s, m >> HB));
+#pragma unroll
+            for (int i = 0; i < NTX; ++i)
+                if (i < s) acc[i] = csub(acc[i], tab(i, s, m));
+        }
+        return acc[0];
+    }
+    template <int N>
+    __device__ __forceinline__ static double bfly_sum(const double (&v)[N]) {
+        double t[N];
+#pragma unroll
+        for (int a = 0; a < N; ++a) t[a] = v[a];
+#pragma unroll
+        for (int o = N / 2; o > 0; o >>= 1)
+#pragma unroll
+            for (int a = 0; a < o; ++a) t[a] = t[a] + t[a + o];
+        return t[0];
+    }
+    template <class Emit>
+    __device__ __forceinline__ static void node_stats(cplx t0, double base, int code, const double* g0, double aref,
+                                                      double inv_s2, Emit emit) {
+        double s[2][3], mn[2];
+#pragma unroll
+        for (int c = 0; c < 2; ++c) {
+            double dd[SQM], w0[SQM], w1[SQM], w2[SQM];
+#pragma unroll
+            for (int a = 0; a < SQM; ++a) dd[a] = sq(c ? t0.y : t0.x, g0[a]);
+            mn[c] = dd[0];
+#pragma unroll
+            for (int a = 1; a < SQM; ++a) mn[c] = fmin(mn[c], dd[a]);
+#pragma unroll
+            for (int a = 0; a < SQM; ++a) {
+                const double pq = pam(a);
+                w0[a] = exp((mn[c] - dd[a]) * inv_s2);
+                w1[a] = __dmul_rn(pq, w0[a]);
+                w2[a] = __dmul_rn(pq * pq, w0[a]);
+            }
+            s[c][0] = bfly_sum(w0);
+            s[c][1] = bfly_sum(w1);
+            s[c][2] = bfly_sum(w2);
+        }
+        const double EI = s[0][0], A1 = s[0][1], A2 = s[0][2], EQ = s[1][0], B1 = s[1][1], B2 = s[1][2];
+        const double W = exp((aref - (base + mn[0] + mn[1])) * inv_s2);
+        const double E0 = __dmul_rn(__dmul_rn(W, EI), EQ);
+        const cplx F0 = mk(__dmul_rn(__dmul_rn(W, A1), EQ), -__dmul_rn(__dmul_rn(W, EI), B1));
+        const double Q0 = __dmul_rn(W, fma(A2, EQ, __dmul_rn(EI, B2)));
+        emit(0, E0);
+        emit(1, F0.x);
+        emit(1 + NTX, F0.y);
+        emit(1 + 2 * NTX, Q0);
+#pragma unroll
+        for (int s_ = 1; s_ < NTX; ++s_) {
+            const cplx xs = cval((code >> (BITS * (NTX - 1 - s_))) & (M - 1));
+            emit(1 + s_, __dmul_rn(E0, xs.x));
+            emit(1 + NTX + s_, -__dmul_rn(E0, xs.y));
+            emit(1 + 2 * NTX + s_, __dmul_rn(E0, cnorm2(xs)));
+            const cplx v = cmul(F0, xs);
+            emit(1 + 3 * NTX + 2 * pair(0, s_), v.x);
+            emit(1 + 3 * NTX + 2 * pair(0, s_) + 1, v.y);
+#pragma unroll
+            for (int i = 1; i < NTX; ++i)
+                if (i < s_) {
+                    const cplx xi = cval((code >> (BITS * (NTX - 1 - i))) & (M - 1));
+                    const cplx cx = cmulc(xs, xi);
+                    emit(1 + 3 * NTX + 2 * pair(i, s_), __dmul_rn(E0, cx.x));
+                    emit(1 + 3 * NTX + 2 * pair(i, s_) + 1, __dmul_rn(E0, cx.y));
+                }
+        }
+    }
+    __device__ __forceinline__ static cplx out_R(const double* A, double invS, int l) {
+        const int i = l / NTX, j = l % NTX;
+        if (i == j) return mk(__dmul_rn(A[1 + 2 * NTX + j], invS), 0.0);
+        const int lo = min(i, j), hi = max(i, j);
+        const int pr = 1 + 3 * NTX + 2 * pair(lo, hi);
+        const double a = __dmul_rn(A[pr], invS), c = __dmul_rn(A[pr + 1], invS);
+        return mk(a, i < j ? c : -c);
+    }
+    __device__ __forceinline__ static cplx out_m(const double* A, double invS, int j) {
+        return mk(__dmul_rn(A[1 + j], invS), __dmul_rn(A[1 + NTX + j], invS));
+    }
+    __device__ __forceinline__ static double out_lse(double aref, double inv_s2, double S) {
+        return fma(-aref, inv_s2, log(S));
     }
 
     __device__ __forceinline__ static double fold(double v, double r) {
@@ -385,6 +530,9 @@
         return a - r;
     }
 };
+
+template <int NTX, int SQM>
+constexpr bool enum_lane_path() { return NTX == 4 && SQM == 4; }
 
 template <int NTX, int SQM>
 __device__ __noinline__ void enum_flush(double* ws, double warp_best) {
@@ -406,82 +554,105 @@
     }
     double* A = ws + E::O_ACC;
     if (n <= 2) {
-        constexpr int LG = (SQM == 2 ? 1 : (SQM == 4 ? 2 : 3));
-        const int a = lane & (SQM - 1);
-        const bool isQ = (lane >> LG) & 1;
-        const double pq = E::pam(a);
-        for (int e = 0; e < n; ++e) {
-            const int code = q[e];
-            double base = ws[E::O_C0];
-            cplx t0;
-            {
-                cplx acc[NTX];
-#pragma unroll
-                for (int i = 0; i < NTX; ++i) acc[i] = mk(ws[E::O_YT + 2 * i], ws[E::O_YT + 2 * i + 1]);
-#pragma unroll
-                for (int s = NTX - 1; s >= 1; --s) {
-                    const int m = (code >> (E::BITS * (NTX - 1 - s))) & (M - 1);
-                    const double eI = acc[s].x - g[s * SQM + (m & (SQM - 1))];
-                    const double eQ = acc[s].y - g[s * SQM + (m >> E::HB)];
-                    base += fma(eI, eI, eQ * eQ);
-#pragma unroll
-                    for (int i = 0; i < NTX; ++i)
-                        if (i < s) acc[i] = csub(acc[i], tab[E::pair(i, s) * M + m]);
+        if constexpr (enum_lane_path<NTX, SQM>()) {
+            cplx yt[NTX];
+#pragma unroll
+            for (int i = 0; i < NTX; ++i) yt[i] = mk(ws[E::O_YT + 2 * i], ws[E::O_YT + 2 * i + 1]);
+            auto tabf = [&](int i, int s, int m) { return tab[E::pair(i, s) * M + m]; };
+            auto lev = [&](int s, int a) { return g[s * SQM + a]; };
+            for (int e = 0; e < n; ++e) {
+                const int code = q[e];
+                double base;
+                const cplx t0 = E::node_residual(yt, ws[E::O_C0], tabf, lev, code, base);
+                constexpr int NR = (E::NACC + 31) / 32;
+                double mine[NR];
+#pragma unroll
+                for (int r = 0; r < NR; ++r) mine[r] = 0.0;
+                E::node_stats(t0, base, code, g, aref, inv_s2,
+                              [&](int idx, double v) { if ((idx & 31) == lane) mine[idx >> 5] = v; });
+#pragma unroll
+                for (int r = 0; r < NR; ++r)
+                    if (32 * r + lane < E::NACC) A[32 * r + lane] += mine[r];
+                __syncwarp();
+            }
+        } else {
+            constexpr int LG = (SQM == 2 ? 1 : (SQM == 4 ? 2 : 3));
+            const int a = lane & (SQM - 1);
+            const bool isQ = (lane >> LG) & 1;
+            const double pq = E::pam(a);
+            for (int e = 0; e < n; ++e) {
+                const int code = q[e];
+                double base = ws[E::O_C0];
+                cplx t0;
+                {
+                    cplx acc[NTX];
+#pragma unroll
+                    for (int i = 0; i < NTX; ++i) acc[i] = mk(ws[E::O_YT + 2 * i], ws[E::O_YT + 2 * i + 1]);
+#pragma unroll
+                    for (int s = NTX - 1; s >= 1; --s) {
+                        const int m = (code >> (E::BITS * (NTX - 1 - s))) & (M - 1);
+                        const double eI = acc[s].x - g[s * SQM + (m & (SQM - 1))];
+                        const double eQ = acc[s].y - g[s * SQM + (m >> E::HB)];
+                        base += fma(eI, eI, eQ * eQ);
+#pragma unroll
+                        for (int i = 0; i < NTX; ++i)
+                            if (i < s) acc[i] = csub(acc[i], tab[E::pair(i, s) * M + m]);
+                    }
+                    t0 = acc[0];
                 }
-                t0 = acc[0];
-            }
-            const double ev = (isQ ? t0.y : t0.x) - g[a];
-            const double dd = ev * ev;
-            double mn = dd;
-#pragma unroll
-            for (int o = SQM / 2; o > 0; o >>= 1) mn = fmin(mn, shfl_xor_d(mn, o));
-            const double w = exp((mn - dd) * inv_s2);
-            double s0 = w, s1 = pq * w, s2 = pq * pq * w;
-#pragma unroll
-            for (int o = SQM / 2; o > 0; o >>= 1) {
-                s0 += shfl_xor_d(s0, o);
-                s1 += shfl_xor_d(s1, o);
-                s2 += shfl_xor_d(s2, o);
-            }
-            const double o0 = shfl_xor_d(s0, SQM), o1 = shfl_xor_d(s1, SQM), o2 = shfl_xor_d(s2, SQM);
-            const double om = shfl_xor_d(mn, SQM);
-            const double EI = isQ ? o0 : s0, A1 = isQ ? o1 : s1, A2 = isQ ? o2 : s2, minI = isQ ? om : mn;
-            const double EQ = isQ ? s0 : o0, B1 = isQ ? s1 : o1, B2 = isQ ? s2 : o2, minQ = isQ ? mn : om;
-            const double W = exp((aref - (base + minI + minQ)) * inv_s2);
-            const double E0 = W * EI * EQ;
-            const cplx F0 = mk(W * A1 * EQ, -W * EI * B1);
-            const double Q0 = W * (A2 * EQ + EI * B2);
-            constexpr int NR = (E::NACC + 31) / 32;
-            double mine[NR];
-#pragma unroll
-            for (int r = 0; r < NR; ++r) mine[r] = 0.0;
-            auto add = [&](int idx, double v) { if ((idx & 31) == lane) mine[idx >> 5] = v; };
-            add(0, E0);
-            add(1, F0.x);
-            add(1 + NTX, F0.y);
-            add(1 + 2 * NTX, Q0);
-#pragma unroll
-            for (int s = 1; s < NTX; ++s) {
-                const cplx xs = E::cval((code >> (E::BITS * (NTX - 1 - s))) & (M - 1));
-                add(1 + s, E0 * xs.x);
-                add(1 + NTX + s, -E0 * xs.y);
-                add(1 + 2 * NTX + s, E0 * cnorm2(xs));
-                const cplx v = cmul(F0, xs);
-                add(1 + 3 * NTX + 2 * E::pair(0, s), v.x);
-                add(1 + 3 * NTX + 2 * E::pair(0, s) + 1, v.y);
-#pragma unroll
-                for (int i = 1; i < NTX; ++i)
-                    if (i < s) {
-                        const cplx xi = E::cval((code >> (E::BITS * (NTX - 1 - i))) & (M - 1));
-                        const cplx cx = cmulc(xs, xi);
-                        add(1 + 3 * NTX + 2 * E::pair(i, s), E0 * cx.x);
-                        add(1 + 3 * NTX + 2 * E::pair(i, s) + 1, E0 * cx.y);
-                    }
-            }
-#pragma unroll
-            for (int r = 0; r < NR; ++r)
-                if (32 * r + lane < E::NACC) A[32 * r + lane] += mine[r];
-            __syncwarp();
+                const double ev = (isQ ? t0.y : t0.x) - g[a];
+                const double dd = ev * ev;
+                double mn = dd;
+#pragma unroll
+                for (int o = SQM / 2; o > 0; o >>= 1) mn = fmin(mn, shfl_xor_d(mn, o));
+                const double w = exp((mn - dd) * inv_s2);
+                double s0 = w, s1 = pq * w, s2 = pq * pq * w;
+#pragma unroll
+                for (int o = SQM / 2; o > 0; o >>= 1) {
+                    s0 += shfl_xor_d(s0, o);
+                    s1 += shfl_xor_d(s1, o);
+                    s2 += shfl_xor_d(s2, o);
+                }
+                const double o0 = shfl_xor_d(s0, SQM), o1 = shfl_xor_d(s1, SQM), o2 = shfl_xor_d(s2, SQM);
+                const double om = shfl_xor_d(mn, SQM);
+                const double EI = isQ ? o0 : s0, A1 = isQ ? o1 : s1, A2 = isQ ? o2 : s2, minI = isQ ? om : mn;
+                const double EQ = isQ ? s0 : o0, B1 = isQ ? s1 : o1, B2 = isQ ? s2 : o2, minQ = isQ ? mn : om;
+                const double W = exp((aref - (base + minI + minQ)) * inv_s2);
+                const double E0 = W * EI * EQ;
+                const cplx F0 = mk(W * A1 * EQ, -W * EI * B1);
+                const double Q0 = W * (A2 * EQ + EI * B2);
+                constexpr int NR = (E::NACC + 31) / 32;
+                double mine[NR];
+#pragma unroll
+                for (int r = 0; r < NR; ++r) mine[r] = 0.0;
+                auto add = [&](int idx, double v) { if ((idx & 31) == lane) mine[idx >> 5] = v; };
+                add(0, E0);
+                add(1, F0.x);
+                add(1 + NTX, F0.y);
+                add(1 + 2 * NTX, Q0);
+#pragma unroll
+                for (int s = 1; s < NTX; ++s) {
+                    const cplx xs = E::cval((code >> (E::BITS * (NTX - 1 - s))) & (M - 1));
+                    add(1 + s, E0 * xs.x);
+                    add(1 + NTX + s, -E0 * xs.y);
+                    add(1 + 2 * NTX + s, E0 * cnorm2(xs));
+                    const cplx v = cmul(F0, xs);
+                    add(1 + 3 * NTX + 2 * E::pair(0, s), v.x);
+                    add(1 + 3 * NTX + 2 * E::pair(0, s) + 1, v.y);
+#pragma unroll
+                    for (int i = 1; i < NTX; ++i)
+                        if (i < s) {
+                            const cplx xi = E::cval((code >> (E::BITS * (NTX - 1 - i))) & (M - 1));
+                            const cplx cx = cmulc(xs, xi);
+                            add(1 + 3 * NTX + 2 * E::pair(i, s), E0 * cx.x);
+                            add(1 + 3 * NTX + 2 * E::pair(i, s) + 1, E0 * cx.y);
+                        }
+                }
+#pragma unroll
+                for (int r = 0; r < NR; ++r)
+                    if (32 * r + lane < E::NACC) A[32 * r + lane] += mine[r];
+                __syncwarp();
+            }
         }
         if (lane == 0) {
             ws[E::O_AREF] = aref;
@@ -588,14 +759,11 @@
     bool prune;
 
     __device__ __forceinline__ void leaf(cplx t0, double nb, int code) {
-        const double fI = E::fold(t0.x, r0), fQ = E::fold(t0.y, r0);
-        const double nodemin = fma(fI, fI, fma(fQ, fQ, nb));
+        const double nodemin = E::nodemin(t0, nb, r0);
         if (nodemin <= lim) {
             if (nodemin <= best) {
-                double dI, dQ;
-                const int iI = E::slice(t0.x, g, dI), iQ = E::slice(t0.y, g, dQ);
-                const double val = nb + dI + dQ;
-                const int k = code + ((iQ * SQM + iI) << (E::BITS * (NTX - 1)));
+                int k;
+                const double val = E::best_leaf(t0, nb, g, code, k);
                 if (val < best || (val == best && k < bestk)) {
                     best = val;
                     bestk = k;
@@ -634,25 +802,20 @@
             const double* g1 = g + SQM;
             double dI1[SQM];
 #pragma unroll
-            for (int a = 0; a < SQM; ++a) {
-                const double eI = acc[1].x - g1[a];
-                dI1[a] = eI * eI;
-            }
+            for (int a = 0; a < SQM; ++a) dI1[a] = E::sq(acc[1].x, g1[a]);
 #pragma unroll 1
             for (int iQ = 0; iQ < SQM; ++iQ) {
-                const double eQ = acc[1].y - g1[iQ];
-                const double bq = base + __dmul_rn(eQ, eQ);
+                const double bq = base + E::sq(acc[1].y, g1[iQ]);
                 const bool deadq = dead || (prune && bq > lim);
                 if (__all_sync(0xffffffffu, deadq)) continue;
                 const double pQ = E::pam(iQ);
-                const cplx tq = mk(fma(pQ, r01.y, acc[0].x), fma(-pQ, r01.x, acc[0].y));
+                const cplx tq = E::sep_row(acc[0], r01, pQ);
                 const int cq = code + ((iQ * SQM) << (E::BITS * (NTX - 2)));
                 if (!deadq) {
 #pragma unroll
                     for (int iI = 0; iI < SQM; ++iI) {
                         const double pI = E::pam(iI);
-                        const cplx t0 = mk(fma(-pI, r01.x, tq.x), fma(-pI, r01.y, tq.y));
-                        leaf(t0, bq + dI1[iI], cq + (iI << (E::BITS * (NTX - 2))));
+                        leaf(E::sep_leaf(tq, r01, pI), bq + dI1[iI], cq + (iI << (E::BITS * (NTX - 2))));
                     }
                 }
                 maybe_flush();
@@ -662,9 +825,7 @@
 #pragma unroll 1
             for (int m = 0; m < M; ++m) {
                 const double* gs = g + S_ * SQM;
-                const double eI = acc[S_].x - gs[m & (SQM - 1)];
-                const double eQ = acc[S_].y - gs[m >> E::HB];
-                const double nb = base + fma(eI, eI, eQ * eQ);
+                const double nb = E::step(base, acc[S_], gs[m & (SQM - 1)], gs[m >> E::HB]);
                 cplx nacc[NTX];
 #pragma unroll
                 for (int i = 0; i < NTX; ++i) nacc[i] = (i < S_) ? csub(acc[i], tab[E::pair(i, S_) * M + m]) : acc[i];
@@ -680,9 +841,7 @@
         } else {
             const int m = (p >> (E::BITS * (LEFT - 1))) & (M - 1);
             const double* gs = g + S_ * SQM;
-            const double eI = acc[S_].x - gs[m & (SQM - 1)];
-            const double eQ = acc[S_].y - gs[m >> E::HB];
-            const double nb = base + fma(eI, eI, eQ * eQ);
+            const double nb = E::step(base, acc[S_], gs[m & (SQM - 1)], gs[m >> E::HB]);
             cplx nacc[NTX];
 #pragma unroll
             for (int i = 0; i < NTX; ++i) nacc[i] = (i < S_) ? csub(acc[i], tab[E::pair(i, S_) * M + m]) : acc[i];
@@ -691,26 +850,20 @@
     }
 };
 
-template <int NTX, int SQM, bool HARD, int WARPS>
-__global__ void __launch_bounds__(WARPS * 32, (NTX > 4 ? 2 : 4)) k_enum(Dims d, const double* __restrict__ qr,
-                                                     const double* __restrict__ varn,
-                                                     const int32_t* __restrict__ active, cplx* __restrict__ stat_m,
-                                                     cplx* __restrict__ stat_R, int32_t* __restrict__ kstar,
-                                                     double* __restrict__ lse_sym) {
+template <int NTX, int SQM, bool HARD>
+__device__ __forceinline__ void enum_symbol(const Dims& d, int b, int t, double* ws, const double* __restrict__ qr,
+                                            const double* __restrict__ varn, const int32_t* __restrict__ active,
+                                            cplx* __restrict__ stat_m, cplx* __restrict__ stat_R,
+                                            int32_t* __restrict__ kstar, double* __restrict__ lse_sym) {
     typedef EnumT<NTX, SQM> E;
     constexpr int M = E::M;
-    extern __shared__ __align__(16) double enum_smem[];
-    const int b = blockIdx.y;
-    const int warp = threadIdx.x >> 5, lane = threadIdx.x & 31;
-    const int t = blockIdx.x * WARPS + warp;
-    if (t >= d.T_d) return;
+    const int lane = threadIdx.x & 31;
     const double* grec = qr + ((size_t)b * d.T_d + t) * d.rec;
     const int32_t act = (active != nullptr) ? active[b] : 1;
     const double vn = varn[b];
     const double rec0 = (lane < d.rec) ? grec[lane] : 0.0;
     if (act == 0) return;
 
-    double* ws = enum_smem + (size_t)warp * E::WS_DOUBLES;
     cplx* tab = (cplx*)(ws + E::O_TAB);
     double* g = ws + E::O_G;
     const double* rec = ws + E::O_SCR;
@@ -750,7 +903,7 @@
 #pragma unroll
             for (int q = 0; q < NTX; ++q)
                 if (q == s) dd = Rm[q][q].x;
-            g[lane] = dd * E::pam(a);
+            g[lane] = __dmul_rn(dd, E::pam(a));
         }
     }
     const double c0 = rec[NTX * (NTX + 1) + 2 * NTX];
@@ -777,22 +930,9 @@
     sc.thr = SBCE_THR * s2;
     sc.prune = (d.flags & SBCE_FLAG_FULL_SCAN) == 0;
     {
-        cplx acc[NTX];
-#pragma unroll
-        for (int i = 0; i < NTX; ++i) acc[i] = yt[i];
-        double base = c0;
-        int k = 0;
-#pragma unroll
-        for (int s = NTX - 1; s >= 0; --s) {
-            double dI, dQ;
-            const int iI = E::slice(acc[s].x, g + s * SQM, dI), iQ = E::slice(acc[s].y, g + s * SQM, dQ);
-            const int m = iQ * SQM + iI;
-            base += dI + dQ;
-            k += m << (E::BITS * (NTX - 1 - s));
-#pragma unroll
-            for (int i = 0; i < NTX; ++i)
-                if (i < s) acc[i] = csub(acc[i], tab[E::pair(i, s) * M + m]);
-        }
+        int k;
+        const double base = E::babai(yt, c0, [&](int i, int s, int m) { return tab[E::pair(i, s) * M + m]; },
+                                     [&](int s, int a) { return g[s * SQM + a]; }, k);
         sc.best = base;
         sc.bestk = k;
         sc.lim = HARD ? base : base + sc.thr;
@@ -804,9 +944,7 @@
         bool a = false;
         if (lane < M) {
             const double* gs = g + (NTX - 1) * SQM;
-            const double eI = yt[NTX - 1].x - gs[lane & (SQM - 1)];
-            const double eQ = yt[NTX - 1].y - gs[lane >> E::HB];
-            a = !(c0 + fma(eI, eI, eQ * eQ) > sc.lim);
+            a = !(E::step(c0, yt[NTX - 1], gs[lane & (SQM - 1)], gs[lane >> E::HB]) > sc.lim);
         }
         top_alive = __ballot_sync(0xffffffffu, a);
     }
@@ -857,22 +995,192 @@
     {
         const double invS = 1.0 / S;
         const double* A = ws + E::O_ACC;
-        for (int l = lane; l < NTX * NTX; l += 32) {
-            const int i = l / NTX, j = l % NTX;
-            cplx v;
-            if (i == j) {
-                v = mk(A[1 + 2 * NTX + j] * invS, 0.0);
-            } else {
-                const int lo = min(i, j), hi = max(i, j);
-                const int pr = 1 + 3 * NTX + 2 * E::pair(lo, hi);
-                const double a = A[pr] * invS, c = A[pr + 1] * invS;
-                v = mk(a, i < j ? c : -c);
-            }
-            stat_R[sidx * NTX * NTX + l] = v;
-        }
-        if (lane < NTX) stat_m[sidx * NTX + lane] = mk(A[1 + lane] * invS, A[1 + NTX + lane] * invS);
-        if (lse_sym != nullptr && lane == 0) lse_sym[sidx] = -ws[E::O_AREF] * inv_s2 + log(S);
-    }
+        for (int l = lane; l < NTX * NTX; l += 32) stat_R[sidx * NTX * NTX + l] = E::out_R(A, invS, l);
+        if (lane < NTX) stat_m[sidx * NTX + lane] = E::out_m(A, invS, lane);
+        if (lse_sym != nullptr && lane == 0) lse_sym[sidx] = E::out_lse(ws[E::O_AREF], inv_s2, S);
+    }
+}
+
+template <int NTX, int SQM, bool HARD, int WARPS>
+__global__ void __launch_bounds__(WARPS * 32, (NTX > 4 ? 2 : 4)) k_enum(Dims d, const double* __restrict__ qr,
+                                                     const double* __restrict__ varn,
+                                                     const int32_t* __restrict__ active, cplx* __restrict__ stat_m,
+                                                     cplx* __restrict__ stat_R, int32_t* __restrict__ kstar,
+                                                     double* __restrict__ lse_sym, const int32_t* __restrict__ dlist,
+                                                     const int32_t* __restrict__ dcount) {
+    extern __shared__ __align__(16) double enum_smem[];
+    const int warp = threadIdx.x >> 5;
+    double* ws = enum_smem + (size_t)warp * EnumT<NTX, SQM>::WS_DOUBLES;
+    if constexpr (HARD || !enum_lane_path<NTX, SQM>()) {
+        const int t = blockIdx.x * WARPS + warp;
+        if (t < d.T_d)
+            enum_symbol<NTX, SQM, HARD>(d, blockIdx.y, t, ws, qr, varn, active, stat_m, stat_R, kstar, lse_sym);
+    } else {
+        const int n = dlist != nullptr ? *dcount : d.T_d;
+        for (int i = blockIdx.x * WARPS + warp; i < n; i += gridDim.x * WARPS) {
+            const int sidx = dlist != nullptr ? dlist[i] : blockIdx.y * d.T_d + i;
+            enum_symbol<NTX, SQM, HARD>(d, sidx / d.T_d, sidx % d.T_d, ws, qr, varn, active, stat_m, stat_R, kstar,
+                                        lse_sym);
+            if (dlist == nullptr) return;
+            __syncwarp();
+        }
+    }
+}
+
+constexpr int ENUM_LANE_BUDGET = 24;
+
+template <int NTX, int SQM>
+struct LaneWalk {
+    typedef EnumT<NTX, SQM> E;
+    static constexpr int M = E::M;
+    static constexpr bool SEP1 = NTX >= 2 && E::PL < NTX - 1;
+    const double* rec;
+    double lim, r0;
+    cplx r01;
+    int live = 0, nq = 0;
+    int qcode = 0;
+    cplx qt0;
+    double qnb = 0.0, qmin = 0.0;
+
+    __device__ __forceinline__ cplx R(int i, int j) const {
+        const int o = 2 * (i * NTX - (i * (i - 1)) / 2 + (j - i));
+        return mk(rec[o], rec[o + 1]);
+    }
+    __device__ __forceinline__ double lev(int s, int a) const { return __dmul_rn(rec[2 * (s * NTX - (s * (s - 1)) / 2)], E::pam(a)); }
+    __device__ __forceinline__ cplx tab(int i, int s, int m) const { return cmul(R(i, s), E::cval(m)); }
+    __device__ __forceinline__ bool over() const { return nq > 1 || live > ENUM_LANE_BUDGET; }
+
+    __device__ __forceinline__ void leaf(cplx t0, double nb, int code) {
+        const double nm = E::nodemin(t0, nb, r0);
+        if (nm <= lim) {
+            ++nq;
+            qcode = code;
+            qt0 = t0;
+            qnb = nb;
+            qmin = nm;
+        }
+    }
+
+    template <int S>
+    __device__ __forceinline__ void walk(const cplx (&acc)[NTX], double base, int code) {
+        if constexpr (S == 0) {
+            leaf(acc[0], base, code);
+        } else if constexpr (S == 1 && SEP1) {
+            double dI1[SQM];
+#pragma unroll
+            for (int a = 0; a < SQM; ++a) dI1[a] = E::sq(acc[1].x, lev(1, a));
+#pragma unroll 1
+            for (int iQ = 0; iQ < SQM; ++iQ) {
+                const double bq = base + E::sq(acc[1].y, lev(1, iQ));
+                if (bq > lim) continue;
+                if (++live > ENUM_LANE_BUDGET) return;
+                const cplx tq = E::sep_row(acc[0], r01, E::pam(iQ));
+                const int cq = code + ((iQ * SQM) << (E::BITS * (NTX - 2)));
+#pragma unroll
+                for (int iI = 0; iI < SQM; ++iI)
+                    leaf(E::sep_leaf(tq, r01, E::pam(iI)), bq + dI1[iI], cq + (iI << (E::BITS * (NTX - 2))));
+                if (nq > 1) return;
+            }
+        } else {
+            unsigned long long alive = 0;
+            {
+                double gs[SQM];
+#pragma unroll
+                for (int a = 0; a < SQM; ++a) gs[a] = lev(S, a);
+#pragma unroll
+                for (int m = 0; m < M; ++m)
+                    if (E::step(base, acc[S], gs[m & (SQM - 1)], gs[m >> E::HB]) <= lim) alive |= 1ull << m;
+            }
+            while (alive != 0ull) {
+                const int m = __ffsll((long long)alive) - 1;
+                alive &= alive - 1ull;
+                const double nb = E::step(base, acc[S], lev(S, m & (SQM - 1)), lev(S, m >> E::HB));
+                if (S > 1 && ++live > ENUM_LANE_BUDGET) return;
+                cplx nacc[NTX];
+#pragma unroll
+                for (int i = 0; i < NTX; ++i) nacc[i] = (i < S) ? csub(acc[i], tab(i, S, m)) : acc[i];
+                walk<S - 1>(nacc, nb, code + (m << (E::BITS * (NTX - 1 - S))));
+                if (over()) return;
+            }
+        }
+    }
+};
+
+template <int NTX, int SQM>
+__global__ void __launch_bounds__(128, 4) k_enum_lane(Dims d, const double* __restrict__ qr,
+                                                      const double* __restrict__ varn,
+                                                      const int32_t* __restrict__ active, cplx* __restrict__ stat_m,
+                                                      cplx* __restrict__ stat_R, int32_t* __restrict__ kstar,
+                                                      double* __restrict__ lse_sym, int32_t* __restrict__ dlist,
+                                                      int32_t* __restrict__ dcount) {
+    typedef EnumT<NTX, SQM> E;
+    constexpr int REC = qr_record_doubles(NTX);
+    constexpr int RS = REC | 1;
+    __shared__ double srec[4][32 * RS];
+    const int b = blockIdx.y;
+    if (active != nullptr && active[b] == 0) return;
+    const int warp = threadIdx.x >> 5, lane = threadIdx.x & 31;
+    const int tw = blockIdx.x * 128 + warp * 32;
+    if (tw >= d.T_d) return;
+    {
+        const int nrec = min(32, d.T_d - tw);
+        const double* g = qr + ((size_t)b * d.T_d + tw) * REC;
+        for (int e = lane; e < nrec * REC; e += 32) srec[warp][(e / REC) * RS + e % REC] = g[e];
+        __syncwarp();
+    }
+    const int t = tw + lane;
+    bool defer = false;
+    if (t < d.T_d) {
+        LaneWalk<NTX, SQM> w;
+        w.rec = &srec[warp][lane * RS];
+        cplx yt[NTX];
+#pragma unroll
+        for (int i = 0; i < NTX; ++i) yt[i] = mk(w.rec[NTX * (NTX + 1) + 2 * i], w.rec[NTX * (NTX + 1) + 2 * i + 1]);
+        const double c0 = w.rec[NTX * (NTX + 1) + 2 * NTX];
+        const double vn = varn[b];
+        const double s2 = vn * vn, inv_s2 = 1.0 / s2;
+        w.r0 = w.rec[0];
+        w.r01 = NTX > 1 ? w.R(0, NTX > 1 ? 1 : 0) : mk(0.0, 0.0);
+        auto tabf = [&](int i, int s, int m) { return w.tab(i, s, m); };
+        auto lev = [&](int s, int a) { return w.lev(s, a); };
+        int bestk;
+        double best = E::babai(yt, c0, tabf, lev, bestk);
+        w.lim = best + SBCE_THR * s2;
+        w.template walk<NTX - 1>(yt, c0, 0);
+        defer = w.over() || w.nq != 1;
+        if (!defer) {
+            double g0[SQM];
+#pragma unroll
+            for (int a = 0; a < SQM; ++a) g0[a] = w.lev(0, a);
+            if (w.qmin <= best) {
+                int k;
+                const double val = E::best_leaf(w.qt0, w.qnb, g0, w.qcode, k);
+                if (val < best || (val == best && k < bestk)) { best = val; bestk = k; }
+            }
+            double base;
+            const cplx t0 = E::node_residual(yt, c0, tabf, lev, w.qcode, base);
+            double A[E::NACC];
+            E::node_stats(t0, base, w.qcode, g0, best, inv_s2, [&](int idx, double v) { A[idx] = 0.0 + v; });
+            const double S = A[0];
+            defer = !(best < 1e300) || !(S > 0.0) || !isfinite(S);
+            if (!defer) {
+                const size_t sidx = (size_t)b * d.T_d + t;
+                const double invS = 1.0 / S;
+#pragma unroll
+                for (int l = 0; l < NTX * NTX; ++l) stat_R[sidx * NTX * NTX + l] = E::out_R(A, invS, l);
+#pragma unroll
+                for (int j = 0; j < NTX; ++j) stat_m[sidx * NTX + j] = E::out_m(A, invS, j);
+                if (kstar != nullptr) kstar[sidx] = bestk;
+                if (lse_sym != nullptr) lse_sym[sidx] = E::out_lse(best, inv_s2, S);
+            }
+        }
+    }
+    const unsigned mask = __ballot_sync(0xffffffffu, defer);
+    if (mask == 0u) return;
+    int base = 0;
+    if (lane == 0) base = atomicAdd(dcount, __popc(mask));
+    base = __shfl_sync(0xffffffffu, base, 0);
+    if (defer) dlist[base + __popc(mask & ((1u << lane) - 1u))] = b * d.T_d + t;
 }
 
 __global__ void k_superimpose_stats(Dims d, int nb, const cplx* __restrict__ Xoff, const int32_t* __restrict__ active,
@@ -944,9 +1252,27 @@
     }
 }
 
+template <int NTX, int SQM, int WARPS>
+static cudaError_t enum_resident_ctas(size_t smem, int* ctas) {
+    static std::atomic<int> have[64];
+    int dev = 0;
+    cudaError_t e = cudaGetDevice(&dev);
+    if (e != cudaSuccess) return e;
+    if (dev >= 0 && dev < 64 && (*ctas = have[dev].load(std::memory_order_relaxed)) > 0) return cudaSuccess;
+    int sms = 0, per_sm = 0;
+    e = cudaDeviceGetAttribute(&sms, cudaDevAttrMultiProcessorCount, dev);
+    if (e == cudaSuccess)
+        e = cudaOccupancyMaxActiveBlocksPerMultiprocessor(&per_sm, k_enum<NTX, SQM, false, WARPS>, WARPS * 32, smem);
+    if (e != cudaSuccess) return e;
+    *ctas = sms * (per_sm > 0 ? per_sm : 1);
+    if (dev >= 0 && dev < 64) have[dev].store(*ctas, std::memory_order_relaxed);
+    return cudaSuccess;
+}
+
 template <int NTX, int SQM>
 static cudaError_t run_enum(const Dims& d, int nb, const double* qr, const double* varn, const int32_t* active,
-                            double* stat_m, double* stat_R, int32_t* kstar, double* lse_sym, cudaStream_t s) {
+                            double* stat_m, double* stat_R, int32_t* kstar, double* lse_sym, int32_t* dlist,
+                            int32_t* dcount, cudaStream_t s) {
     constexpr int WARPS = 4;
     dim3 grid((d.T_d + WARPS - 1) / WARPS, nb);
     constexpr size_t smem = sizeof(double) * WARPS * EnumT<NTX, SQM>::WS_DOUBLES;
@@ -956,14 +1282,35 @@
         e = opt_in_smem(optin_hard, (const void*)k_enum<NTX, SQM, true, WARPS>, smem);
         if (e != cudaSuccess) return e;
         k_enum<NTX, SQM, true, WARPS><<<grid, WARPS * 32, smem, s>>>(d, qr, varn, active, (cplx*)stat_m,
-                                                                      (cplx*)stat_R, kstar, lse_sym);
-    } else {
-        e = opt_in_smem(optin_soft, (const void*)k_enum<NTX, SQM, false, WARPS>, smem);
+                                                                      (cplx*)stat_R, kstar, lse_sym, nullptr, nullptr);
+        count_launch();
+        return cudaGetLastError();
+    }
+    e = opt_in_smem(optin_soft, (const void*)k_enum<NTX, SQM, false, WARPS>, smem);
+    if (e != cudaSuccess) return e;
+    if (!enum_lane_path<NTX, SQM>() || (d.flags & SBCE_FLAG_FULL_SCAN)) {
+        k_enum<NTX, SQM, false, WARPS><<<grid, WARPS * 32, smem, s>>>(d, qr, varn, active, (cplx*)stat_m,
+                                                                       (cplx*)stat_R, kstar, lse_sym, nullptr, nullptr);
+        count_launch();
+        return cudaGetLastError();
+    }
+    if constexpr (enum_lane_path<NTX, SQM>()) {
+        int ctas = 0;
+        e = enum_resident_ctas<NTX, SQM, WARPS>(smem, &ctas);
         if (e != cudaSuccess) return e;
-        k_enum<NTX, SQM, false, WARPS><<<grid, WARPS * 32, smem, s>>>(d, qr, varn, active, (cplx*)stat_m,
-                                                                       (cplx*)stat_R, kstar, lse_sym);
-    }
-    count_launch();
+        e = cudaMemsetAsync(dcount, 0, sizeof(int32_t), s);
+        if (e != cudaSuccess) return e;
+        k_enum_lane<NTX, SQM><<<dim3((d.T_d + 127) / 128, nb), 128, 0, s>>>(d, qr, varn, active, (cplx*)stat_m,
+                                                                            (cplx*)stat_R, kstar, lse_sym, dlist,
+                                                                            dcount);
+        count_launch();
+        e = cudaGetLastError();
+        if (e != cudaSuccess) return e;
+        const long long worst = ((long long)nb * d.T_d + WARPS - 1) / WARPS;
+        k_enum<NTX, SQM, false, WARPS><<<(unsigned)std::min<long long>(ctas, worst), WARPS * 32, smem, s>>>(
+            d, qr, varn, active, (cplx*)stat_m, (cplx*)stat_R, kstar, lse_sym, dlist, dcount);
+        count_launch();
+    }
     return cudaGetLastError();
 }
 
@@ -979,21 +1326,23 @@
 
 template <int NTX>
 static cudaError_t run_enum_wide(const Dims& d, int nb, const double* qr, const double* varn, const int32_t* active,
-                                 double* stat_m, double* stat_R, int32_t* kstar, double* lse_sym, cudaStream_t s) {
-    if (d.sqM == 2) return run_enum<NTX, 2>(d, nb, qr, varn, active, stat_m, stat_R, kstar, lse_sym, s);
+                                 double* stat_m, double* stat_R, int32_t* kstar, double* lse_sym, int32_t* dlist,
+                                 int32_t* dcount, cudaStream_t s) {
+    if (d.sqM == 2) return run_enum<NTX, 2>(d, nb, qr, varn, active, stat_m, stat_R, kstar, lse_sym, dlist, dcount, s);
     if constexpr (NTX <= 6) {
-        if (d.sqM == 4) return run_enum<NTX, 4>(d, nb, qr, varn, active, stat_m, stat_R, kstar, lse_sym, s);
+        if (d.sqM == 4) return run_enum<NTX, 4>(d, nb, qr, varn, active, stat_m, stat_R, kstar, lse_sym, dlist, dcount, s);
     }
     return cudaErrorInvalidValue;
 }
 
 template <int NTX>
 static cudaError_t run_enum_ntx(const Dims& d, int nb, const double* qr, const double* varn, const int32_t* active,
-                                double* stat_m, double* stat_R, int32_t* kstar, double* lse_sym, cudaStream_t s) {
+                                double* stat_m, double* stat_R, int32_t* kstar, double* lse_sym, int32_t* dlist,
+                                int32_t* dcount, cudaStream_t s) {
     switch (d.sqM) {
-        case 2: return run_enum<NTX, 2>(d, nb, qr, varn, active, stat_m, stat_R, kstar, lse_sym, s);
-        case 4: return run_enum<NTX, 4>(d, nb, qr, varn, active, stat_m, stat_R, kstar, lse_sym, s);
-        case 8: return run_enum<NTX, 8>(d, nb, qr, varn, active, stat_m, stat_R, kstar, lse_sym, s);
+        case 2: return run_enum<NTX, 2>(d, nb, qr, varn, active, stat_m, stat_R, kstar, lse_sym, dlist, dcount, s);
+        case 4: return run_enum<NTX, 4>(d, nb, qr, varn, active, stat_m, stat_R, kstar, lse_sym, dlist, dcount, s);
+        case 8: return run_enum<NTX, 8>(d, nb, qr, varn, active, stat_m, stat_R, kstar, lse_sym, dlist, dcount, s);
         default: return cudaErrorInvalidValue;
     }
 }
@@ -1014,16 +1363,17 @@
 }
 
 cudaError_t launch_enum(const Dims& d, int nb, const double* qr, const double* varn, const int32_t* active,
-                        double* stat_m, double* stat_R, int32_t* kstar, double* lse_sym, cudaStream_t s) {
+                        double* stat_m, double* stat_R, int32_t* kstar, double* lse_sym, int32_t* dlist,
+                        int32_t* dcount, cudaStream_t s) {
     switch (d.n_tx) {
-        case 1: return run_enum_ntx<1>(d, nb, qr, varn, active, stat_m, stat_R, kstar, lse_sym, s);
-        case 2: return run_enum_ntx<2>(d, nb, qr, varn, active, stat_m, stat_R, kstar, lse_sym, s);
-        case 3: return run_enum_ntx<3>(d, nb, qr, varn, active, stat_m, stat_R, kstar, lse_sym, s);
-        case 4: return run_enum_ntx<4>(d, nb, qr, varn, active, stat_m, stat_R, kstar, lse_sym, s);
-        case 5: return run_enum_wide<5>(d, nb, qr, varn, active, stat_m, stat_R, kstar, lse_sym, s);
-        case 6: return run_enum_wide<6>(d, nb, qr, varn, active, stat_m, stat_R, kstar, lse_sym, s);
-        case 7: return run_enum_wide<7>(d, nb, qr, varn, active, stat_m, stat_R, kstar, lse_sym, s);
-        case 8: return run_enum_wide<8>(d, nb, qr, varn, active, stat_m, stat_R, kstar, lse_sym, s);
+        case 1: return run_enum_ntx<1>(d, nb, qr, varn, active, stat_m, stat_R, kstar, lse_sym, dlist, dcount, s);
+        case 2: return run_enum_ntx<2>(d, nb, qr, varn, active, stat_m, stat_R, kstar, lse_sym, dlist, dcount, s);
+        case 3: return run_enum_ntx<3>(d, nb, qr, varn, active, stat_m, stat_R, kstar, lse_sym, dlist, dcount, s);
+        case 4: return run_enum_ntx<4>(d, nb, qr, varn, active, stat_m, stat_R, kstar, lse_sym, dlist, dcount, s);
+        case 5: return run_enum_wide<5>(d, nb, qr, varn, active, stat_m, stat_R, kstar, lse_sym, dlist, dcount, s);
+        case 6: return run_enum_wide<6>(d, nb, qr, varn, active, stat_m, stat_R, kstar, lse_sym, dlist, dcount, s);
+        case 7: return run_enum_wide<7>(d, nb, qr, varn, active, stat_m, stat_R, kstar, lse_sym, dlist, dcount, s);
+        case 8: return run_enum_wide<8>(d, nb, qr, varn, active, stat_m, stat_R, kstar, lse_sym, dlist, dcount, s);
         default: return cudaErrorInvalidValue;
     }
 }
```

Measured after the change: 26830, median of 6. 1.15x the previous value.
